# Nikhil-Kulkarni/RayTrace-miniapp

Measured on AMD Instinct MI355X. Metric: ray_steps_per_sec, higher is better.
Workload: dtype f32+f64

## Files before the change

### include/rt_hip.h

```cpp
#ifndef RT_HIP_H
#define RT_HIP_H

#include <stddef.h>
#include <stdint.h>

#ifdef __cplusplus
extern "C" {
#endif

#define RT_N_SUB 3
#define RT_N_FAILED_MAX 32
#define RT_N_SEED_MAX 2

enum {
    RT_OK            = 0,
    RT_ERR_ARG       = 1,
    RT_ERR_NO_DEVICE = 2,
    RT_ERR_HIP       = 3,
    RT_ERR_NOMEM     = 4
};

typedef struct rt_ray {
    float x, y, a, b;
} rt_ray;
// ... 38 lines not shown

int rt_hip_device_count(void);

const char *rt_hip_last_error(void);

int rt_hip_selftest(int device, unsigned long long *n_checked, unsigned long long *n_mismatch);

int rt_hip_image_loop(int device, int N, const rt_beam *beam, const rt_gain *gain,
                      const rt_seed *seed, int method, const rt_ray *rays, size_t n_rays,
                      double scale, double *image, double *I_ang, unsigned int *failure_code,
                      rt_ray *failed_rays, int max_failed, int *n_failed, rt_stats *stats);

int rt_hip_multi_image_loop(int ndev, int N, const rt_beam *beam, const rt_gain *gain, const rt_seed *seed,
                            int method, const rt_ray *rays, size_t n_rays, double scale, double *image,
                            double *I_ang, unsigned int *failure_code, rt_ray *failed_rays, int max_failed,
                            int *n_failed, rt_stats *stats);

int rt_hip_ray_list_grid_dims(const rt_ray *rays, size_t n_rays, int dims[4]);

int rt_hip_multi_last_mode(void);

int rt_hip_host_libm_mode(int device);

void rt_hip_pool_trim(void);

typedef struct rt_hip_plan rt_hip_plan;

int rt_hip_plan_create(rt_hip_plan **plan, int device, int N, const rt_beam *beam,
                       const rt_gain *gain, const rt_seed *seed, int method, double scale);

int rt_hip_plan_set_rays(rt_hip_plan *plan, const rt_ray *rays, size_t n_rays);

int rt_hip_plan_set_ray_grid(rt_hip_plan *plan, const double *gx, int ngx, const double *gy,
                             int ngy, const double *ga, int nga, const double *gb, int ngb,
                             int64_t first, int64_t stride, int64_t count);

int rt_hip_plan_run(rt_hip_plan *plan, void *stream, double *image_dev, double *iang_dev);

int rt_hip_plan_fetch(rt_hip_plan *plan, double *image, double *I_ang,
                      unsigned int *failure_code, rt_ray *failed_rays, int max_failed,
                      int *n_failed, rt_stats *stats);

int rt_hip_plan_kernel_ms(rt_hip_plan *plan, float *ms);

int rt_hip_plan_kernel_times(rt_hip_plan *plan, float *march_ms, float *freq_ms);

int rt_hip_plan_last_fused(rt_hip_plan *plan);

int rt_hip_plan_last_march_instance(rt_hip_plan *plan);

typedef struct rt_hip_run_facts {
    unsigned size;
    int cu_count;
    unsigned long long lds_limit, n_rays, blob_bytes, n_iang;
    unsigned n_tiles;
    int K, Kp, L, rays_per_pixel, n_seed, march_prune, method;
    float c_h3;
    unsigned safe, debug;
    int use_emis, own_cells, exclusive, path_on, spectra_on, step_on, step_one_launch, probe_on, has_ray_list, host_rays,
        tables_bounded, ntest_proven, gv_has_nan;
    int occupancy_per_cu;
    int scan_on;
} rt_hip_run_facts;
typedef struct rt_hip_run_shape {
    unsigned size;
    int kind, lds_tab;
    unsigned n_launch, bthr;
    int mode, bounded, opt, last_march_inst;
    unsigned long long mlds;
    unsigned grid, chunk, park, spin_limit, no_skip, late_first, late_waves, late_chunks;
    int occupancy_asked;
    int maxq, nslot;
    unsigned off_exp, off_iang, off_ctl, off_rem, off_nodes, off_buf, node_cap, n_free, per_wave, split, k_part, n_consumers,
        consumers_first;
    unsigned long long flds, tile_links;
    unsigned fgrid;
    int key_s6, key_emis, key_excl;
    int pass_kind, pass_wg_waves, pass_in_lds, pass_nslot;
    unsigned long long pass_lds;
    unsigned pass_grid, pass_fetch_shift;
} rt_hip_run_shape;
int rt_hip_debug_run_shape(const rt_hip_run_facts *facts, rt_hip_run_shape *out);

int rt_hip_plan_set_timing_ring(rt_hip_plan *plan, int n_runs);
int rt_hip_plan_ring_times(rt_hip_plan *plan, float *march_ms, float *freq_ms, int max_runs, int *n_runs);

double *rt_hip_plan_image_ptr(rt_hip_plan *plan);
double *rt_hip_plan_iang_ptr(rt_hip_plan *plan);

int rt_hip_plan_enable_probe(rt_hip_plan *plan, int on);
int rt_hip_plan_fetch_probe(rt_hip_plan *plan, float *gvl, float *evl, int32_t *ivl,
                            rt_ray *ray2, uint32_t *flags, uint32_t *steps);

int rt_hip_plan_set_exact_emission(rt_hip_plan *plan, int on);

int rt_hip_plan_set_step_factor(rt_hip_plan *plan, double c);

int rt_hip_plan_enable_path(rt_hip_plan *plan, int on);
int rt_hip_plan_fetch_path(rt_hip_plan *plan, float *path, int32_t *err);

int rt_hip_plan_enable_spectra(rt_hip_plan *plan, int on);
int rt_hip_plan_fetch_spectra(rt_hip_plan *plan, double *Iv, rt_ray *ray2, int32_t *err);
double *rt_hip_plan_spectra_ptr(rt_hip_plan *plan);

int rt_hip_plan_enable_length_spectra(rt_hip_plan *plan, int on);
int rt_hip_plan_fetch_length_spectra(rt_hip_plan *plan, int n, double *Iv, rt_ray *ray2, int32_t *err);
int rt_hip_plan_length_spectra_ptrs(rt_hip_plan *plan, int n, double **Iv_dev, rt_ray **ray2_dev, int32_t **err_dev);

int rt_hip_plan_set_spectra_seeds(rt_hip_plan *plan, int n_seed, const rt_seed *seeds);
int rt_hip_plan_fetch_seed_spectra(rt_hip_plan *plan, int s, double *Iv, rt_ray *ray2, int32_t *err);
int rt_hip_plan_seed_spectra_ptrs(rt_hip_plan *plan, int s, double **Iv_dev, rt_ray **ray2_dev, int32_t **err_dev);
int rt_hip_plan_fetch_seed_length_spectra(rt_hip_plan *plan, int s, int n, double *Iv, rt_ray *ray2, int32_t *err);
int rt_hip_plan_seed_length_spectra_ptrs(rt_hip_plan *plan, int s, int n, double **Iv_dev, rt_ray **ray2_dev, int32_t **err_dev);

int rt_hip_plan_set_spectra_ase_seeds(rt_hip_plan *plan, int n_seed, const rt_seed *seeds);
int rt_hip_plan_fetch_full_spectra(rt_hip_plan *plan, int r, double *Iv, rt_ray *ray2, int32_t *err);
int rt_hip_plan_full_spectra_ptrs(rt_hip_plan *plan, int r, double **Iv_dev, rt_ray **ray2_dev, int32_t **err_dev);

int rt_hip_plan_set_length_spectra_ase_seeds(rt_hip_plan *plan, int n_seed, const rt_seed *seeds);
int rt_hip_plan_fetch_full_length_spectra(rt_hip_plan *plan, int r, int n, double *Iv, rt_ray *ray2, int32_t *err);
int rt_hip_plan_full_length_spectra_ptrs(rt_hip_plan *plan, int r, int n, double **Iv_dev, rt_ray **ray2_dev, int32_t **err_dev);

int rt_hip_calc_rays(int device, int N, double dz, const rt_gain *gain, const rt_seed *seed, int K, int method,
                     const double *rays, size_t n, double *Iv, double *ray2, int32_t *err, rt_stats *stats);

int rt_hip_plan_enable_step(rt_hip_plan *plan, int on);
int rt_hip_plan_set_step_buffers(rt_hip_plan *plan, double *E_v_dev, double *nf_dev);
int rt_hip_plan_fetch_step(rt_hip_plan *plan, double *E_v, double *nf, double *I_ang);
int rt_hip_plan_step_ptrs(rt_hip_plan *plan, double **E_v_dev, double **nf_dev);
int rt_hip_multi_step_loop(int ndev, int N, const rt_beam *beam, const rt_gain *gain, const rt_seed *seed, int method,
                           const rt_ray *rays, size_t n_rays, double scale, double *E_v, double *nf, double *I_ang,
                           unsigned int *failure_code, rt_ray *failed_rays, int max_failed, int *n_failed, rt_stats *stats);
int rt_hip_step_loop(int device, int N, const rt_beam *beam, const rt_gain *gain, const rt_seed *seed, int method,
                     const rt_ray *rays, size_t n_rays, double scale, double *E_v, double *nf, double *I_ang,
                     unsigned int *failure_code, rt_ray *failed_rays, int max_failed, int *n_failed, rt_stats *stats);

int rt_hip_plan_set_step_one_launch(rt_hip_plan *plan, int on);

typedef struct rt_gain_values {
    const double *n;
    const float *g0;
    const float *E0;
    const float *gv;
} rt_gain_values;
int rt_hip_plan_update_gain(rt_hip_plan *plan, int N, const rt_gain_values *vals);
int rt_hip_plan_update_gain_dev(rt_hip_plan *plan, int N, const rt_gain_values *vals, void *stream);
int rt_hip_plan_table_flags(rt_hip_plan *plan, int *bounded, int *ntest_proven, int *gv_nonfinite, float *gs_cap);

int rt_hip_plan_set_seeds(rt_hip_plan *plan, int n_seed, const rt_seed *seeds);
int rt_hip_plan_fetch_seed_step(rt_hip_plan *plan, int s, double *E_v, double *nf, double *I_ang,
                                unsigned int *failure_code);
int rt_hip_plan_seed_step_ptrs(rt_hip_plan *plan, int s, double **E_v_dev, double **nf_dev, double **iang_dev);

#define RT_N_SCAN_MAX 32
int rt_hip_plan_enable_length_scan(rt_hip_plan *plan, int on);
int rt_hip_plan_fetch_length_step(rt_hip_plan *plan, int n, double *E_v, double *nf, double *I_ang, unsigned int *failure_code);
int rt_hip_plan_length_step_ptrs(rt_hip_plan *plan, int n, double **E_v_dev, double **nf_dev, double **iang_dev);
int rt_hip_length_scan_loop(int device, int N, const rt_beam *beam, const rt_gain *gain, const rt_seed *seed, int method,
                            const rt_ray *rays, size_t n_rays, double scale, double *E_v, double *nf, double *I_ang,
                            unsigned int *failure_codes, rt_ray *failed_rays, int max_failed, int *n_failed, rt_stats *stats);

int rt_hip_plan_enable_suffix_scan(rt_hip_plan *plan, int on);
int rt_hip_suffix_scan_loop(int device, int N, const rt_beam *beam, const rt_gain *gain, const rt_seed *seed, int method,
                            const rt_ray *rays, size_t n_rays, double scale, double *E_v, double *nf, double *I_ang,
                            unsigned int *failure_codes, rt_ray *failed_rays, int max_failed, int *n_failed, rt_stats *stats);

// ... 71 lines not shown
```

### raytrace-miniapp_amd/backend.py

```python
from __future__ import annotations

import ctypes as C
import subprocess
import time
from pathlib import Path

import numpy as np

from . import cabi
from .problem import Problem, Seed

CSRC = Path(__file__).resolve().parent / "csrc"
LIB_PATH = CSRC / "librt_hip.so"


class RayTraceError(RuntimeError):
    """Raised where the reference calls RAY_ERROR (utilities/RayUtilityMacros.h:88-91)."""


def build_library(force: bool = False) -> Path:
    if force and LIB_PATH.exists():
        LIB_PATH.unlink()
    subprocess.run(["make", "-s", "-C", str(CSRC)], check=True)
    return LIB_PATH
# ... 579 lines not shown
            U, B = C.POINTER(C.c_uint), C.POINTER(C.c_ubyte)
            self.hl.check(self.hl.lib.rt_hip_plan_history_fetch(
                self._h, r, cabi._dp(E_v), cabi._dp(nf), cabi._dp(iang), cabi._dp(es), code.ctypes.data_as(U),
                flags.ctypes.data_as(U), filled.ctypes.data_as(B)), "rt_hip_plan_history_fetch")
            out.append(dict(E_v=E_v, nf=nf, I_ang=iang, E_sum=es, failure_code=code, flags=flags, filled=filled))
        return out

    def fetch_history_sum(self) -> list:
        b, out = self.problem.beam, []
        for r in range(max(1, self.history_info()["n_rec"])):
            E_v, nf, iang, es = np.empty(b.nv), np.empty(b.nx * b.ny), np.empty(b.na * b.nb), np.empty(1)
            self.hl.check(self.hl.lib.rt_hip_plan_history_fetch_sum(self._h, r, cabi._dp(E_v), cabi._dp(nf), cabi._dp(iang),
                                                                    cabi._dp(es)), "rt_hip_plan_history_fetch_sum")
            out.append(dict(E_v=E_v, nf=nf, I_ang=iang, E_sum=float(es[0])))
        return out

    def history_tensors(self) -> list:
        import torch

        b, info, out = self.problem.beam, self.history_info(), []
        T = info["n_steps"]
        for r in range(info["n_rec"]):
            q = [C.c_void_p() for _ in range(6)]
            self.hl.check(self.hl.lib.rt_hip_plan_history_ptrs(self._h, r, *(C.byref(x) for x in q)), "rt_hip_plan_history_ptrs")
            e, n, a, s, c, f = (int(x.value or 0) for x in q)
            words = lambda ptr: _view(ptr, (T // 2 + T % 2,), self.device).view(torch.int32)[:T]
            out.append(dict(E_v=_view(e, (T, b.nv), self.device), nf=_view(n, (T, b.ny, b.nx), self.device),
                            I_ang=_view(a, (T, b.nb, b.na), self.device), E_sum=_view(s, (T,), self.device),
                            failure_code=words(c), flags=words(f)))
        return out

    def history_sum_tensors(self) -> list:
        out = []
        for r in range(self.history_info()["n_rec"]):
            q = [C.c_void_p() for _ in range(4)]
            self.hl.check(self.hl.lib.rt_hip_plan_history_sum_ptrs(self._h, r, *(C.byref(x) for x in q)), "rt_hip_plan_history_sum_ptrs")
            e, n, a, s = (int(x.value or 0) for x in q)
            out.append(dict(**self._record_views((e, n, a)), E_sum=_view(s, (1,), self.device)))
        return out

    def update_gain(self, gain, stream: int | None = None) -> "Plan":
        import copy
        import dataclasses

        old = self.problem.gain
        gv = cabi.GainValues(gain, [(g.Nx, g.Ny) for g in old], self.problem.beam.nv, self.device)
        if gv.on_device:
            if stream is None:
                import torch
                stream = torch.cuda.current_stream(self.device).cuda_stream
            rc = self.hl.lib.rt_hip_plan_update_gain_dev(self._h, gv.N, gv.vals, C.c_void_p(stream))
            self.hl.check(rc, "rt_hip_plan_update_gain_dev")
            self._gain_dev = gv
        else:
            self.hl.check(self.hl.lib.rt_hip_plan_update_gain(self._h, gv.N, gv.vals), "rt_hip_plan_update_gain")
            q = copy.copy(self.problem)
            q.gain = [old[0]] + [dataclasses.replace(old[i], n=t[0], g0=t[1], E0=t[2], gv=t[3]) for i, t in enumerate(gv.tables) if i]
            q.golden_image = q.golden_I_ang = None
            self.problem = q
        return self

    def table_flags(self) -> dict:
        b, t, g, cap = C.c_int(0), C.c_int(0), C.c_int(0), C.c_float(0)
        self.hl.check(self.hl.lib.rt_hip_plan_table_flags(self._h, C.byref(b), C.byref(t), C.byref(g), C.byref(cap)),
                      "rt_hip_plan_table_flags")
        return dict(bounded=b.value, ntest_proven=t.value, gv_nonfinite=g.value, gs_cap=np.float32(cap.value))

    def kernel_ms(self) -> float:
        ms = C.c_float(0)
        self.hl.check(self.hl.lib.rt_hip_plan_kernel_ms(self._h, C.byref(ms)), "rt_hip_plan_kernel_ms")
        return float(ms.value)

    def kernel_times(self) -> tuple:
        a, f = C.c_float(0), C.c_float(0)
        self.hl.check(self.hl.lib.rt_hip_plan_kernel_times(self._h, C.byref(a), C.byref(f)),
                      "rt_hip_plan_kernel_times")
        return float(a.value), float(f.value)

    def last_fused(self) -> bool:
        return bool(self.hl.lib.rt_hip_plan_last_fused(self._h))

    def last_march_instance(self) -> int:
        return int(self.hl.lib.rt_hip_plan_last_march_instance(self._h))

    def set_timing_ring(self, n_runs: int) -> "Plan":
        self.hl.check(self.hl.lib.rt_hip_plan_set_timing_ring(self._h, int(n_runs)), "rt_hip_plan_set_timing_ring")
        self._ring = int(n_runs)
        return self

    def ring_times(self) -> list:
        n = self._ring
        if n < 1:
            return []
        a = np.zeros(n, np.float32)
        f = np.zeros(n, np.float32)
        got = C.c_int(0)
        self.hl.check(self.hl.lib.rt_hip_plan_ring_times(self._h, cabi._fp(a), cabi._fp(f), n, C.byref(got)),
                      "rt_hip_plan_ring_times")
        return [(float(a[i]), float(f[i])) for i in range(got.value)]

    def fetch_probe(self) -> dict:
        n = self.n_rays
        S = (self.problem.N - 1) * cabi.RT_N_SUB
        out = dict(gvl=np.zeros((n, S), np.float32), evl=np.zeros((n, S), np.float32),
                   ivl=np.zeros((n, S), np.int32), ray2=np.zeros(n, cabi.RAY_DTYPE),
                   flags=np.zeros(n, np.uint32), steps=np.zeros(n, np.uint32))
        P = C.POINTER
        rc = self.hl.lib.rt_hip_plan_fetch_probe(
            self._h, cabi._fp(out["gvl"]), cabi._fp(out["evl"]), out["ivl"].ctypes.data_as(P(C.c_int32)),
            cabi.rays_ptr(out["ray2"]), out["flags"].ctypes.data_as(P(C.c_uint32)),
            out["steps"].ctypes.data_as(P(C.c_uint32)))
        self.hl.check(rc, "rt_hip_plan_fetch_probe")
        return out

    @property
    def image_ptr(self) -> int:
        return int(self.hl.lib.rt_hip_plan_image_ptr(self._h) or 0)

    @property
    def iang_ptr(self) -> int:
        return int(self.hl.lib.rt_hip_plan_iang_ptr(self._h) or 0)

    def close(self) -> None:
        if self._h:
            self.hl.lib.rt_hip_plan_destroy(self._h)
            self._h = C.c_void_p()

    def __enter__(self):
        return self

    def __exit__(self, *exc):
        self.close()

    def __del__(self):
        try:
            self.close()
        except Exception:
            pass


def _host_loop(entry: str, problem: Problem, rays, device: int, lead: tuple = (), seeds=None, scales=None, ase: bool = False,
               image: bool = False) -> dict:
    hl = HipLibrary.get()
    m = cabi.Marshalled(problem)
    if rays is None:
        rays = problem.build_rays()
    rays = np.ascontiguousarray(rays, dtype=cabi.RAY_DTYPE)
    b = problem.beam
    sizes = (b.nx * b.ny * b.nv, b.na * b.nb) if image else (b.nv, b.nx * b.ny, b.na * b.nb)
    outs = [np.zeros(lead + (n,)) for n in sizes]
    codes = np.zeros(lead, np.uint32)
    nfail = C.c_int(0)
    failed = np.zeros(cabi.RT_N_FAILED_MAX, dtype=cabi.RAY_DTYPE)
    st = cabi.RtStats()
    args = [device, m.N, C.byref(m.beam), m.gain] + ([] if ase else [m.seed_ref])
    args += [problem.method, cabi.rays_ptr(rays), len(rays), problem.scale]
    if seeds is not None:
        _, arr, _keep = _seed_array(seeds, entry, "a call")
        args += [len(seeds), arr] + ([cabi._dp(scales) if scales is not None else None] if ase else [])
    args += [cabi._dp(o) for o in outs] + [codes.ctypes.data_as(C.POINTER(C.c_uint)), cabi.rays_ptr(failed), cabi.RT_N_FAILED_MAX,
                                          C.byref(nfail), C.byref(st)]
    t0 = time.perf_counter()
    rc = getattr(hl.lib, entry)(*args)
    call_ms = (time.perf_counter() - t0) * 1e3
    hl.check(rc, entry)
    return dict(outs=outs, codes=codes, failure_code=int(np.bitwise_or.reduce(codes, axis=None)), failed_rays=failed[:nfail.value].copy(),
# ... 288 lines not shown
```

### raytrace-miniapp_amd/cabi.py

```python
from __future__ import annotations

import ctypes as C

import numpy as np

RT_N_SUB = 3
RT_N_FAILED_MAX = 32
RT_N_SEED_MAX = 2
RT_N_SCAN_MAX = 32

RT_OK, RT_ERR_ARG, RT_ERR_NO_DEVICE, RT_ERR_HIP, RT_ERR_NOMEM = range(5)

c_double_p = C.POINTER(C.c_double)
c_float_p = C.POINTER(C.c_float)


class RtRay(C.Structure):
    _fields_ = [("x", C.c_float), ("y", C.c_float), ("a", C.c_float), ("b", C.c_float)]


RAY_DTYPE = np.dtype([("x", "<f4"), ("y", "<f4"), ("a", "<f4"), ("b", "<f4")])


class RtBeam(C.Structure):
# ... 252 lines not shown
                                             C.c_int64, C.c_int64, C.c_int64]
    lib.rt_hip_plan_set_ray_grid.restype = C.c_int
    lib.rt_hip_plan_run.argtypes = [vp, vp, vp, vp]
    lib.rt_hip_plan_run.restype = C.c_int
    lib.rt_hip_plan_fetch.argtypes = [vp, c_double_p, c_double_p, P(C.c_uint), P(RtRay), C.c_int,
                                      P(C.c_int), P(RtStats)]
    lib.rt_hip_plan_fetch.restype = C.c_int
    lib.rt_hip_plan_kernel_ms.argtypes = [vp, P(C.c_float)]
    lib.rt_hip_plan_kernel_ms.restype = C.c_int
    lib.rt_hip_plan_kernel_times.argtypes = [vp, P(C.c_float), P(C.c_float)]
    lib.rt_hip_plan_kernel_times.restype = C.c_int
    lib.rt_hip_plan_last_fused.argtypes = [vp]
    lib.rt_hip_plan_last_fused.restype = C.c_int
    if hasattr(lib, "rt_hip_plan_last_march_instance"):
        lib.rt_hip_plan_last_march_instance.argtypes = [vp]
        lib.rt_hip_plan_last_march_instance.restype = C.c_int
    lib.rt_hip_plan_set_timing_ring.argtypes = [vp, C.c_int]
    lib.rt_hip_plan_set_timing_ring.restype = C.c_int
    lib.rt_hip_plan_ring_times.argtypes = [vp, c_float_p, c_float_p, C.c_int, P(C.c_int)]
    lib.rt_hip_plan_ring_times.restype = C.c_int
    lib.rt_hip_plan_image_ptr.argtypes = [vp]
    lib.rt_hip_plan_image_ptr.restype = vp
    lib.rt_hip_plan_iang_ptr.argtypes = [vp]
    lib.rt_hip_plan_iang_ptr.restype = vp
    lib.rt_hip_plan_enable_probe.argtypes = [vp, C.c_int]
    lib.rt_hip_plan_enable_probe.restype = C.c_int
    lib.rt_hip_plan_fetch_probe.argtypes = [vp, c_float_p, c_float_p, P(C.c_int32), P(RtRay),
                                            P(C.c_uint32), P(C.c_uint32)]
    lib.rt_hip_plan_fetch_probe.restype = C.c_int
    lib.rt_hip_plan_set_exact_emission.argtypes = [vp, C.c_int]
    lib.rt_hip_plan_set_exact_emission.restype = C.c_int
    lib.rt_hip_plan_set_step_factor.argtypes = [vp, C.c_double]
    lib.rt_hip_plan_set_step_factor.restype = C.c_int
    lib.rt_hip_plan_enable_path.argtypes = [vp, C.c_int]
    lib.rt_hip_plan_enable_path.restype = C.c_int
    lib.rt_hip_plan_fetch_path.argtypes = [vp, c_float_p, P(C.c_int32)]
    lib.rt_hip_plan_fetch_path.restype = C.c_int
    lib.rt_hip_plan_enable_spectra.argtypes = [vp, C.c_int]
    lib.rt_hip_plan_enable_spectra.restype = C.c_int
    lib.rt_hip_plan_fetch_spectra.argtypes = [vp, c_double_p, P(RtRay), P(C.c_int32)]
    lib.rt_hip_plan_fetch_spectra.restype = C.c_int
    lib.rt_hip_plan_spectra_ptr.argtypes = [vp]
    lib.rt_hip_plan_spectra_ptr.restype = vp
    lib.rt_hip_calc_rays.argtypes = [C.c_int, C.c_int, C.c_double, P(RtGain), P(RtSeed), C.c_int, C.c_int, c_double_p,
                                     C.c_size_t, c_double_p, c_double_p, P(C.c_int32), P(RtStats)]
    lib.rt_hip_calc_rays.restype = C.c_int
    if hasattr(lib, "rt_hip_plan_enable_step"):
        lib.rt_hip_plan_enable_step.argtypes = [vp, C.c_int]
        lib.rt_hip_plan_enable_step.restype = C.c_int
        lib.rt_hip_plan_fetch_step.argtypes = [vp, c_double_p, c_double_p, c_double_p]
        lib.rt_hip_plan_fetch_step.restype = C.c_int
        lib.rt_hip_plan_step_ptrs.argtypes = [vp, P(vp), P(vp)]
        lib.rt_hip_plan_step_ptrs.restype = C.c_int
        lib.rt_hip_step_loop.argtypes = [
            C.c_int, C.c_int, P(RtBeam), P(RtGain), P(RtSeed), C.c_int, P(RtRay), C.c_size_t,
            C.c_double, c_double_p, c_double_p, c_double_p, P(C.c_uint), P(RtRay), C.c_int, P(C.c_int),
            P(RtStats)]
        lib.rt_hip_step_loop.restype = C.c_int
    if hasattr(lib, "rt_hip_multi_step_loop"):
        lib.rt_hip_plan_set_step_buffers.argtypes = [vp, vp, vp]
        lib.rt_hip_plan_set_step_buffers.restype = C.c_int
        lib.rt_hip_multi_step_loop.argtypes = list(lib.rt_hip_step_loop.argtypes)
        lib.rt_hip_multi_step_loop.restype = C.c_int
    if hasattr(lib, "rt_hip_plan_update_gain"):
        lib.rt_hip_plan_update_gain.argtypes = [vp, C.c_int, P(RtGainValues)]
        lib.rt_hip_plan_update_gain.restype = C.c_int
        lib.rt_hip_plan_update_gain_dev.argtypes = [vp, C.c_int, P(RtGainValues), vp]
        lib.rt_hip_plan_update_gain_dev.restype = C.c_int
        lib.rt_hip_plan_table_flags.argtypes = [vp, P(C.c_int), P(C.c_int), P(C.c_int), c_float_p]
        lib.rt_hip_plan_table_flags.restype = C.c_int
    if hasattr(lib, "rt_hip_plan_set_seeds"):
        lib.rt_hip_plan_set_seeds.argtypes = [vp, C.c_int, P(RtSeed)]
        lib.rt_hip_plan_set_seeds.restype = C.c_int
        lib.rt_hip_plan_fetch_seed_step.argtypes = [vp, C.c_int, c_double_p, c_double_p, c_double_p, P(C.c_uint)]
        lib.rt_hip_plan_fetch_seed_step.restype = C.c_int
        lib.rt_hip_plan_seed_step_ptrs.argtypes = [vp, C.c_int, P(vp), P(vp), P(vp)]
        lib.rt_hip_plan_seed_step_ptrs.restype = C.c_int
    if hasattr(lib, "rt_hip_plan_set_step_one_launch"):
        lib.rt_hip_plan_set_step_one_launch.argtypes = [vp, C.c_int]
        lib.rt_hip_plan_set_step_one_launch.restype = C.c_int
    if hasattr(lib, "rt_hip_debug_run_shape"):
        lib.rt_hip_debug_run_shape.argtypes = [P(RtRunFacts), P(RtRunShape)]
        lib.rt_hip_debug_run_shape.restype = C.c_int
    if hasattr(lib, "rt_hip_plan_enable_length_scan"):
        lib.rt_hip_plan_enable_length_scan.argtypes = [vp, C.c_int]
        lib.rt_hip_plan_enable_length_scan.restype = C.c_int
        lib.rt_hip_plan_fetch_length_step.argtypes = [vp, C.c_int, c_double_p, c_double_p, c_double_p, P(C.c_uint)]
        lib.rt_hip_plan_fetch_length_step.restype = C.c_int
        lib.rt_hip_plan_length_step_ptrs.argtypes = [vp, C.c_int, P(vp), P(vp), P(vp)]
        lib.rt_hip_plan_length_step_ptrs.restype = C.c_int
        lib.rt_hip_length_scan_loop.argtypes = list(lib.rt_hip_step_loop.argtypes)
        lib.rt_hip_length_scan_loop.restype = C.c_int
    if hasattr(lib, "rt_hip_plan_enable_suffix_scan"):
        lib.rt_hip_plan_enable_suffix_scan.argtypes = [vp, C.c_int]
        lib.rt_hip_plan_enable_suffix_scan.restype = C.c_int
        lib.rt_hip_suffix_scan_loop.argtypes = list(lib.rt_hip_step_loop.argtypes)
        lib.rt_hip_suffix_scan_loop.restype = C.c_int
    if hasattr(lib, "rt_hip_plan_set_scan_seeds"):
        lib.rt_hip_plan_set_scan_seeds.argtypes = [vp, C.c_int, P(RtSeed)]
        lib.rt_hip_plan_set_scan_seeds.restype = C.c_int
        lib.rt_hip_plan_fetch_seed_length_step.argtypes = [vp, C.c_int, C.c_int, c_double_p, c_double_p, c_double_p, P(C.c_uint)]
        lib.rt_hip_plan_fetch_seed_length_step.restype = C.c_int
        lib.rt_hip_plan_seed_length_step_ptrs.argtypes = [vp, C.c_int, C.c_int, P(vp), P(vp), P(vp)]
        lib.rt_hip_plan_seed_length_step_ptrs.restype = C.c_int
        a = list(lib.rt_hip_step_loop.argtypes)
        lib.rt_hip_seed_length_scan_loop.argtypes = a[:9] + [C.c_int, P(RtSeed)] + a[9:]
        lib.rt_hip_seed_length_scan_loop.restype = C.c_int
    if hasattr(lib, "rt_hip_plan_set_ase_seeds"):
        lib.rt_hip_plan_set_ase_seeds.argtypes = [vp, C.c_int, P(RtSeed), c_double_p]
        lib.rt_hip_plan_set_ase_seeds.restype = C.c_int
        lib.rt_hip_plan_fetch_full_step.argtypes = [vp, C.c_int, c_double_p, c_double_p, c_double_p, P(C.c_uint)]
        lib.rt_hip_plan_fetch_full_step.restype = C.c_int
        lib.rt_hip_plan_full_step_ptrs.argtypes = [vp, C.c_int, P(vp), P(vp), P(vp)]
        lib.rt_hip_plan_full_step_ptrs.restype = C.c_int
        lib.rt_hip_full_step_loop.argtypes = [
            C.c_int, C.c_int, P(RtBeam), P(RtGain), C.c_int, P(RtRay), C.c_size_t, C.c_double, C.c_int, P(RtSeed), c_double_p,
            c_double_p, c_double_p, c_double_p, P(C.c_uint), P(RtRay), C.c_int, P(C.c_int), P(RtStats)]
        lib.rt_hip_full_step_loop.restype = C.c_int
    if hasattr(lib, "rt_hip_plan_set_scan_ase_seeds"):
        lib.rt_hip_plan_set_scan_ase_seeds.argtypes = [vp, C.c_int, P(RtSeed), c_double_p]
        lib.rt_hip_plan_set_scan_ase_seeds.restype = C.c_int
        lib.rt_hip_plan_fetch_full_length_step.argtypes = [vp, C.c_int, C.c_int, c_double_p, c_double_p, c_double_p, P(C.c_uint)]
        lib.rt_hip_plan_fetch_full_length_step.restype = C.c_int
        lib.rt_hip_plan_full_length_step_ptrs.argtypes = [vp, C.c_int, C.c_int, P(vp), P(vp), P(vp)]
        lib.rt_hip_plan_full_length_step_ptrs.restype = C.c_int
        lib.rt_hip_full_length_scan_loop.argtypes = list(lib.rt_hip_full_step_loop.argtypes)
        lib.rt_hip_full_length_scan_loop.restype = C.c_int
    if hasattr(lib, "rt_hip_plan_set_suffix_ase_seeds"):
        lib.rt_hip_plan_set_suffix_ase_seeds.argtypes = [vp, C.c_int, P(RtSeed), c_double_p]
        lib.rt_hip_plan_set_suffix_ase_seeds.restype = C.c_int
        lib.rt_hip_full_suffix_scan_loop.argtypes = list(lib.rt_hip_full_length_scan_loop.argtypes)
        lib.rt_hip_full_suffix_scan_loop.restype = C.c_int
    if hasattr(lib, "rt_hip_plan_set_suffix_seeds"):
        lib.rt_hip_plan_set_suffix_seeds.argtypes = list(lib.rt_hip_plan_set_scan_seeds.argtypes)
        lib.rt_hip_plan_set_suffix_seeds.restype = C.c_int
        lib.rt_hip_seed_suffix_scan_loop.argtypes = list(lib.rt_hip_seed_length_scan_loop.argtypes)
        lib.rt_hip_seed_suffix_scan_loop.restype = C.c_int
    if hasattr(lib, "rt_hip_plan_enable_length_spectra"):
        lib.rt_hip_plan_enable_length_spectra.argtypes = [vp, C.c_int]
        lib.rt_hip_plan_enable_length_spectra.restype = C.c_int
        lib.rt_hip_plan_fetch_length_spectra.argtypes = [vp, C.c_int, c_double_p, P(RtRay), P(C.c_int32)]
        lib.rt_hip_plan_fetch_length_spectra.restype = C.c_int
        lib.rt_hip_plan_length_spectra_ptrs.argtypes = [vp, C.c_int, P(vp), P(vp), P(vp)]
        lib.rt_hip_plan_length_spectra_ptrs.restype = C.c_int
    if hasattr(lib, "rt_hip_plan_set_spectra_seeds"):
        lib.rt_hip_plan_set_spectra_seeds.argtypes = [vp, C.c_int, P(RtSeed)]
        lib.rt_hip_plan_set_spectra_seeds.restype = C.c_int
        lib.rt_hip_plan_fetch_seed_spectra.argtypes = [vp, C.c_int, c_double_p, P(RtRay), P(C.c_int32)]
        lib.rt_hip_plan_fetch_seed_spectra.restype = C.c_int
        lib.rt_hip_plan_seed_spectra_ptrs.argtypes = [vp, C.c_int, P(vp), P(vp), P(vp)]
        lib.rt_hip_plan_seed_spectra_ptrs.restype = C.c_int
        lib.rt_hip_plan_fetch_seed_length_spectra.argtypes = [vp, C.c_int, C.c_int, c_double_p, P(RtRay), P(C.c_int32)]
        lib.rt_hip_plan_fetch_seed_length_spectra.restype = C.c_int
        lib.rt_hip_plan_seed_length_spectra_ptrs.argtypes = [vp, C.c_int, C.c_int, P(vp), P(vp), P(vp)]
        lib.rt_hip_plan_seed_length_spectra_ptrs.restype = C.c_int
    if hasattr(lib, "rt_hip_plan_set_spectra_ase_seeds"):
        lib.rt_hip_plan_set_spectra_ase_seeds.argtypes = [vp, C.c_int, P(RtSeed)]
        lib.rt_hip_plan_set_spectra_ase_seeds.restype = C.c_int
        lib.rt_hip_plan_fetch_full_spectra.argtypes = [vp, C.c_int, c_double_p, P(RtRay), P(C.c_int32)]
        lib.rt_hip_plan_fetch_full_spectra.restype = C.c_int
        lib.rt_hip_plan_full_spectra_ptrs.argtypes = [vp, C.c_int, P(vp), P(vp), P(vp)]
        lib.rt_hip_plan_full_spectra_ptrs.restype = C.c_int
    if hasattr(lib, "rt_hip_plan_set_length_spectra_ase_seeds"):
        lib.rt_hip_plan_set_length_spectra_ase_seeds.argtypes = [vp, C.c_int, P(RtSeed)]
        lib.rt_hip_plan_set_length_spectra_ase_seeds.restype = C.c_int
        lib.rt_hip_plan_fetch_full_length_spectra.argtypes = [vp, C.c_int, C.c_int, c_double_p, P(RtRay), P(C.c_int32)]
        lib.rt_hip_plan_fetch_full_length_spectra.restype = C.c_int
        lib.rt_hip_plan_full_length_spectra_ptrs.argtypes = [vp, C.c_int, C.c_int, P(vp), P(vp), P(vp)]
        lib.rt_hip_plan_full_length_spectra_ptrs.restype = C.c_int
    if hasattr(lib, "rt_hip_plan_history_create"):
        up, bp = P(C.c_uint), P(C.c_ubyte)
        lib.rt_hip_plan_history_create.argtypes = [vp, C.c_int]
        lib.rt_hip_plan_history_create.restype = C.c_int
        lib.rt_hip_plan_history_append.argtypes = [vp, C.c_int, C.c_double, C.c_int, vp]
        lib.rt_hip_plan_history_append.restype = C.c_int
        lib.rt_hip_plan_history_ptrs.argtypes = [vp, C.c_int, P(vp), P(vp), P(vp), P(vp), P(vp), P(vp)]
        lib.rt_hip_plan_history_ptrs.restype = C.c_int
        lib.rt_hip_plan_history_sum_ptrs.argtypes = [vp, C.c_int, P(vp), P(vp), P(vp), P(vp)]
        lib.rt_hip_plan_history_sum_ptrs.restype = C.c_int
        lib.rt_hip_plan_history_fetch.argtypes = [vp, C.c_int, c_double_p, c_double_p, c_double_p, c_double_p, up, up, bp]
        lib.rt_hip_plan_history_fetch.restype = C.c_int
        lib.rt_hip_plan_history_fetch_sum.argtypes = [vp, C.c_int, c_double_p, c_double_p, c_double_p, c_double_p]
        lib.rt_hip_plan_history_fetch_sum.restype = C.c_int
        lib.rt_hip_plan_history_info.argtypes = [vp, P(C.c_int), P(C.c_int), P(C.c_int)]
        lib.rt_hip_plan_history_info.restype = C.c_int
        lib.rt_hip_debug_history_layout.argtypes = [P(RtHistoryFacts), P(RtHistoryLayout)]
        lib.rt_hip_debug_history_layout.restype = C.c_int
    lib.rt_hip_plan_set_debug.argtypes = [vp, C.c_uint]
    lib.rt_hip_plan_set_debug.restype = C.c_int
    lib.rt_hip_plan_destroy.argtypes = [vp]
    lib.rt_hip_plan_destroy.restype = None


HIP_API_SYMBOLS = [
    "rt_hip_device_count", "rt_hip_last_error", "rt_hip_selftest", "rt_hip_image_loop", "rt_hip_multi_image_loop",
    "rt_hip_multi_last_mode", "rt_hip_ray_list_grid_dims", "rt_hip_host_libm_mode", "rt_hip_pool_trim", "rt_hip_plan_create",
    "rt_hip_plan_set_rays", "rt_hip_plan_set_ray_grid", "rt_hip_plan_run", "rt_hip_plan_fetch",
    "rt_hip_plan_kernel_ms", "rt_hip_plan_kernel_times", "rt_hip_plan_last_fused", "rt_hip_plan_last_march_instance", "rt_hip_plan_set_timing_ring", "rt_hip_plan_ring_times", "rt_hip_plan_image_ptr", "rt_hip_plan_iang_ptr", "rt_hip_plan_enable_probe",
    "rt_hip_plan_fetch_probe", "rt_hip_plan_set_exact_emission", "rt_hip_plan_set_step_factor", "rt_hip_plan_enable_path",
    "rt_hip_plan_fetch_path", "rt_hip_plan_enable_spectra", "rt_hip_plan_fetch_spectra", "rt_hip_plan_spectra_ptr",
    "rt_hip_calc_rays", "rt_hip_plan_enable_step", "rt_hip_plan_fetch_step", "rt_hip_plan_step_ptrs", "rt_hip_step_loop",
    "rt_hip_plan_set_step_buffers", "rt_hip_multi_step_loop",
    "rt_hip_plan_update_gain", "rt_hip_plan_update_gain_dev", "rt_hip_plan_table_flags",
    "rt_hip_plan_set_seeds", "rt_hip_plan_fetch_seed_step", "rt_hip_plan_seed_step_ptrs",
    "rt_hip_plan_enable_length_scan", "rt_hip_plan_fetch_length_step", "rt_hip_plan_length_step_ptrs", "rt_hip_length_scan_loop",
    "rt_hip_plan_set_scan_seeds", "rt_hip_plan_fetch_seed_length_step", "rt_hip_plan_seed_length_step_ptrs",
    "rt_hip_seed_length_scan_loop",
    "rt_hip_plan_enable_suffix_scan", "rt_hip_suffix_scan_loop",
    "rt_hip_plan_set_ase_seeds", "rt_hip_plan_fetch_full_step", "rt_hip_plan_full_step_ptrs", "rt_hip_full_step_loop",
    "rt_hip_plan_set_scan_ase_seeds", "rt_hip_plan_fetch_full_length_step", "rt_hip_plan_full_length_step_ptrs",
    "rt_hip_full_length_scan_loop",
    "rt_hip_plan_set_suffix_ase_seeds", "rt_hip_full_suffix_scan_loop",
    "rt_hip_plan_set_suffix_seeds", "rt_hip_seed_suffix_scan_loop",
    "rt_hip_plan_enable_length_spectra", "rt_hip_plan_fetch_length_spectra", "rt_hip_plan_length_spectra_ptrs",
    "rt_hip_plan_set_spectra_seeds", "rt_hip_plan_fetch_seed_spectra", "rt_hip_plan_seed_spectra_ptrs",
    "rt_hip_plan_fetch_seed_length_spectra", "rt_hip_plan_seed_length_spectra_ptrs",
    "rt_hip_plan_set_spectra_ase_seeds", "rt_hip_plan_fetch_full_spectra", "rt_hip_plan_full_spectra_ptrs",
    "rt_hip_plan_set_length_spectra_ase_seeds", "rt_hip_plan_fetch_full_length_spectra", "rt_hip_plan_full_length_spectra_ptrs",
    "rt_hip_plan_set_step_one_launch", "rt_hip_debug_run_shape",
    "rt_hip_plan_history_create", "rt_hip_plan_history_append", "rt_hip_plan_history_ptrs", "rt_hip_plan_history_sum_ptrs",
    "rt_hip_plan_history_fetch", "rt_hip_plan_history_fetch_sum", "rt_hip_plan_history_info", "rt_hip_debug_history_layout",
    "rt_hip_plan_set_debug", "rt_hip_plan_destroy",
]
```

### raytrace-miniapp_amd/csrc/rt_blob_pack.h

```cpp
#pragma once

#include <cmath>
#include <cstring>
#include <vector>

#include "rt_device.h"

namespace rt {

inline BlobGain blob_pack_length(std::vector<unsigned char> &blob, size_t i, int Nx, int Ny, const double *x, const double *y,
                                 const double *n, const float *g0, const float *E0, bool &tiny_spacing, bool &bad_index)
{
    const size_t npix = (size_t) Nx * (size_t) Ny;
    BlobGain h;
    memset(&h, 0, sizeof(h));
    h.lo_x     = (float) x[0];
    h.hi_x     = (float) x[Nx - 1];
    h.lo_y     = (float) y[0];
    h.hi_y     = (float) y[Ny - 1];
    h.mirror_y = 0;
    if (h.lo_y >= 0) {
        h.lo_y     = -h.hi_y;
        h.mirror_y = 1;
    }
    h.Nx  = Nx;
    h.Ny  = Ny;
    h.x0f = (float) x[0];
    h.y0f = (float) y[0];
    const double ihx = (double) (Nx - 1) / (x[Nx - 1] - x[0]);
    const double ihy = (double) (Ny - 1) / (y[Ny - 1] - y[0]);
    h.inv_hxf        = std::isfinite(ihx) && fabs(ihx) < 1e30 ? (float) ihx : 0.0f;
    h.inv_hyf        = std::isfinite(ihy) && fabs(ihy) < 1e30 ? (float) ihy : 0.0f;
    auto put_intervals = [&](const double *gp, int n, bool mirrored) {
        const int off = (int) blob.size();
        blob.resize(blob.size() + sizeof(Interval) * (size_t) n);
        Interval *iv = reinterpret_cast<Interval *>(blob.data() + off);
        memset(iv, 0, sizeof(Interval) * (size_t) n);
        for (int k = 1; k < n; k++) {
            const double lo = gp[k - 1], hi = gp[k], hk = hi - lo;
            if (!(hk >= 1e-30))
                tiny_spacing = true;
            iv[k].lo   = lo;
            iv[k].hi   = hi;
            iv[k].rh   = 1.0 / hk;
            iv[k].rw   = 1.0 / (double) (float) hk;
            iv[k].w    = (float) hk;
            iv[k].b_lo = (float) (lo - 0.1 * hk);
            iv[k].b_hi = (float) (hi + 0.1 * hk);
            if (mirrored && k == 1)
                iv[k].b_lo = -iv[k].b_hi;
        }
        return off;
    };
    h.off_ix   = put_intervals(x, Nx, false);
    h.off_iy   = put_intervals(y, Ny, h.mirror_y != 0);
    h.off_node = (int) blob.size();
    blob.resize(blob.size() + sizeof(Node) * npix);
    Node *nd = reinterpret_cast<Node *>(blob.data() + h.off_node);
    for (size_t c = 0; c < npix; c++) {
        if (!std::isfinite((float) n[c]))
            bad_index = true;
        nd[c].n  = n[c];
        nd[c].g0 = g0[c];
        nd[c].E0 = E0 ? E0[c] : 0.0f;
    }
    memcpy(blob.data() + sizeof(BlobGain) * i, &h, sizeof(h));
    return h;
}

}
```

### raytrace-miniapp_amd/csrc/rt_device.h

```cpp
#pragma once

#include <hip/hip_runtime.h>
#include <stdint.h>

#include "../../include/rt_hip.h"

namespace rt {

constexpr int WAVE = 64;

struct alignas(16) Node {
    double n;
    float g0;
    float E0;
};

struct DevGain {
    const float *gv;
};

struct alignas(16) BlobGain {
    float lo_x, hi_x, lo_y, hi_y;
    int Nx, Ny, mirror_y, off_ix;
    int off_iy, off_node, pad0, pad1;
    float x0f, y0f;
    float inv_hxf, inv_hyf;
};

struct alignas(16) Interval {
    double lo;
    double rw;
    float w;
    float b_lo;
    float b_hi;
    float pad;
    double hi;
    double rh;
};

struct DevSeed {
    const double *x[5];
    const double *f[5];
    int dim[5];
    int pad;
    double f0;
};

struct DevBeam {
    const double *x, *y, *a, *b, *dv;
    int nx, ny, na, nb, nv;
    int pad;
    double dx, dy, da, db;
    double inv_dx, inv_dy, inv_da, inv_db;
    double g_first[4], g_last[4];
};

struct DevRays {
    const rt_ray *list;
    const float *sxy;
    const double *gx, *gy, *ga, *gb;
    const float *tan_a, *tan_b;
    const double *sf;
    const unsigned char *sin;
    int ngx, ngy, nga, ngb;
    long long first, stride;
    unsigned long long count;
    unsigned div_mul[3], div_sh[3];
};

struct RecSlot {
    float g, e;
    int c;
};
struct RecMeta {
    float px, py, sx, sy, sz;
    unsigned flags_steps;
};

struct DevCtl {
    unsigned int next_tile[8][8][16];
    unsigned int next_tile_f[4][8][16];
    unsigned int failure_code;
    unsigned int n_failed;
    unsigned long long cell_steps;
    unsigned long long n_escaped;
    unsigned long long n_skipped;
    unsigned long long n_rays;
    rt_ray failed[RT_N_FAILED_MAX];
    unsigned int seed_code[RT_N_SEED_MAX];
    unsigned int len_code[RT_N_SCAN_MAX];
    unsigned int seed_len_code[RT_N_SEED_MAX][RT_N_SCAN_MAX];
    unsigned int rec_code[RT_N_SEED_MAX + 2];
    unsigned int rec_len_code[1 + RT_N_SEED_MAX][RT_N_SCAN_MAX];
};

struct DevProbe {
    rt_ray *ray2;
    uint32_t *flags;
    uint32_t *steps;
};

struct DevParams {
    int N, L, K, method;
    int use_emis, has_seed;
    float dz0;
    int probe_on;
    int Kp;
    int exact_emis;
    double scale;
    DevBeam beam;
    DevSeed seed;
    const DevGain *gain;
    DevRays rays;
    double *image;
    double *iang;
    DevCtl *ctl;
    DevProbe probe;
    unsigned int n_tiles;
    unsigned int tile_begin, tile_end, freq_id;
    unsigned int ray_begin, ray_end, launch_id, pad_launch;
    unsigned int debug;
// ... 103 lines not shown
```

### raytrace-miniapp_amd/csrc/rt_launch.hip

```cpp
#include "rt_path.hip"
#include "rt_freq.hip"
#include "rt_fused.hip"
#include "rt_spec.hip"
#include "rt_step.hip"
#include "rt_step_seeds.hip"
#include "rt_fused_step.hip"
#include "rt_step_scan.hip"
#include "rt_step_rscan.hip"
#include "rt_step_scan_seeds.hip"
#include "rt_step_ase_seeds.hip"
#include "rt_step_scan_ase_seeds.hip"
#include "rt_step_rscan_ase_seeds.hip"

#include "rt_step_rscan_seeds.hip"
#include "rt_spec_scan.hip"
#include "rt_spec_seeds.hip"
#include "rt_spec_scan_seeds.hip"
#include "rt_spec_ase_seeds.hip"
#include "rt_spec_scan_ase_seeds.hip"

#include "rt_runtime.h"
#include "rt_run_shape.h"

#include <atomic>
// ... 103 lines not shown
void (*step_kernel(bool s6, bool emis))(const rt::StepKArg)
{
    return emis ? (s6 ? rt::rt_step_kernel<6, true> : rt::rt_step_kernel<0, true>) : (s6 ? rt::rt_step_kernel<6, false> : rt::rt_step_kernel<0, false>);
}
void (*seeds_kernel(bool s6))(const rt::SeedsKArg) { return s6 ? rt::rt_step_seeds_kernel<6> : rt::rt_step_seeds_kernel<0>; }
void (*ase_seeds_kernel(bool s6))(const rt::AseSeedsKArg) { return s6 ? rt::rt_step_ase_seeds_kernel<6> : rt::rt_step_ase_seeds_kernel<0>; }
void (*scan_kernel(bool emis))(const rt::ScanKArg) { return emis ? rt::rt_step_scan_kernel<true> : rt::rt_step_scan_kernel<false>; }
void (*rscan_kernel(bool emis))(const rt::ScanKArg) { return emis ? rt::rt_step_rscan_kernel<true> : rt::rt_step_rscan_kernel<false>; }
void (*spec_scan_kernel(bool emis, bool backward))(const rt::SpecScanKArg)
{
    return emis ? (backward ? rt::rt_spec_scan_kernel<true, true> : rt::rt_spec_scan_kernel<true, false>)
                : (backward ? rt::rt_spec_scan_kernel<false, true> : rt::rt_spec_scan_kernel<false, false>);
}
void (*spec_seeds_kernel(bool s6))(const rt::SpecSeedsKArg) { return s6 ? rt::rt_spec_seeds_kernel<6> : rt::rt_spec_seeds_kernel<0>; }
void (*spec_ase_seeds_kernel(bool s6))(const rt::SpecSeedsKArg) { return s6 ? rt::rt_spec_ase_seeds_kernel<6> : rt::rt_spec_ase_seeds_kernel<0>; }
void (*spec_scan_seeds_kernel(bool backward))(const rt::SpecScanSeedsKArg)
{
    return backward ? rt::rt_spec_scan_seeds_kernel<true> : rt::rt_spec_scan_seeds_kernel<false>;
}
void (*spec_scan_ase_seeds_kernel(bool backward))(const rt::SpecScanSeedsKArg)
{
    return backward ? rt::rt_spec_scan_ase_seeds_kernel<true> : rt::rt_spec_scan_ase_seeds_kernel<false>;
}

struct PassRun {
    unsigned tile_begin, tile_end, freq_id;
    unsigned safe;
    unsigned char *bad;
};

rt::FreqKArg freq_args(const rt_hip_plan *p, bool iang_in_lds, int nslot, unsigned fetch_shift, const PassRun &r)
{
    const rt::DevParams &P = p->P;
    rt::FreqKArg a;
    memset(&a, 0, sizeof(a));
    a.hot.gv0        = p->gv_dev.size() > 1 ? p->gv_dev[1] : nullptr;
    a.hot.gv1        = p->gv_dev.size() > 2 ? p->gv_dev[2] : nullptr;
    a.hot.gain       = P.gain;
    a.hot.rec        = P.rec;
    a.hot.image      = P.image;
    a.hot.iang       = P.iang;
    a.hot.ctl        = P.ctl;
    a.hot.dv2        = p->dv2_dev;
    a.hot.seed_fk    = P.has_seed ? P.seed.f[4] : p->dv2_dev;
    a.hot.bad        = r.bad;
    a.hot.scale      = P.scale;
    a.hot.gs_cap     = P.gs_cap;
    a.hot.K          = P.K;
    a.hot.Kp         = P.Kp;
    a.hot.L          = P.L;
    a.hot.method     = P.method;
    a.hot.rec_stride = P.rec_stride;
    a.hot.n_rays     = (unsigned) P.rays.count;
    a.hot.tile_begin = r.tile_begin;
    a.hot.tile_end   = r.tile_end;
    a.hot.freq_id    = r.freq_id;
    a.hot.fetch_shift = fetch_shift;
    a.hot.nslot      = nslot;
    a.hot.nx         = P.beam.nx;
    a.hot.ny         = P.beam.ny;
    a.hot.n_ang      = P.beam.na * P.beam.nb;
    a.hot.flags      = (P.exclusive ? rt::FQ_EXCLUSIVE : 0u) | (r.safe == 1 ? rt::FQ_SAFE_CHECK : 0u) |
                  (r.safe == 2 ? rt::FQ_SAFE_SKIP : 0u) | (P.exact_emis ? rt::FQ_EXACT_EMIS : 0u) |
                  (P.has_seed ? rt::FQ_HAS_SEED : 0u) | (P.probe_on ? rt::FQ_PROBE : 0u) |
                  (p->gv_has_nan ? rt::FQ_GV_NAN : 0u) | (iang_in_lds ? rt::FQ_IANG_LDS : 0u) |
                  ((P.method != 1 || P.has_seed || P.probe_on) ? rt::FQ_NEED_EXIT : 0u) |
                  (P.own_cells ? rt::FQ_OWN_CELLS : 0u) | ((P.debug & 4u) ? rt::FQ_DBG_NOFLUSH : 0u);
    a.cold.beam  = P.beam;
    a.cold.seed  = P.seed;
    a.cold.rays  = P.rays;
    a.cold.probe = P.probe;
    return a;
}

RunFacts run_facts(const rt_hip_plan *p)
{
    const rt::DevParams &P = p->P;
    RunFacts f;
    f.cu_count        = p->cu_count;
    f.lds_limit       = p->lds_limit;
    f.n_rays          = p->n_rays;
    f.n_tiles         = P.n_tiles;
    f.blob_bytes      = P.blob_bytes;
    f.K               = P.K;
    f.Kp              = P.Kp;
    f.L               = P.L;
    f.n_iang          = p->n_iang;
    f.rays_per_pixel  = P.rays.nga * P.rays.ngb;
    f.n_seed          = p->scan_on ? p->n_scan_seed : p->n_seed;
    if (p->n_spec_seed > 0)
        f.n_seed = p->n_spec_seed;
    f.c_h3            = P.c_h3;
    f.march_prune     = p->march_prune;
    f.method          = P.method;
    f.safe            = P.safe;
    f.debug           = P.debug;
    f.use_emis        = P.use_emis != 0;
    f.own_cells       = P.own_cells != 0;
    f.exclusive       = P.exclusive != 0;
    f.path_on         = p->path_on;
    f.spectra_on      = p->spectra_on;
    f.step_on         = p->step_on;
    f.step_one_launch = p->step_one_launch;
    f.probe_on        = p->probe_on;
    f.has_ray_list    = P.rays.list != nullptr;
    f.host_rays       = p->host_rays != nullptr;
    f.tables_bounded  = p->tables_bounded;
    f.ntest_proven    = p->ntest_proven;
    f.gv_has_nan      = p->gv_has_nan;
    f.scan_on         = p->scan_on && p->step_on;
    f.length_spectra_on = p->lspec_on;
    return f;
}

template <typename KArg> KArg pass_args(const rt::FreqKArg &fa)
{
    KArg a;
    memset(&a, 0, sizeof(a));
    a.hot       = fa.hot;
    a.hot.image = nullptr;
    a.cold      = fa.cold;
    return a;
}

rt::SeedRec seed_rec(const rt_hip_plan *p, int r)
{
    double *blk = p->recs_dev + (size_t) r * p->recs_stride;
    return rt::SeedRec{ blk, blk + p->recs_nf_off, blk + p->recs_ang_off };
}
void fill_scan(rt::ScanArg &a, const rt_hip_plan *p) { a = rt::ScanArg{ p->scan_bnd, p->recs_dev, p->recs_stride, p->recs_nf_off, p->recs_ang_off }; }
int fill_seed_tabs(rt::SeedTabs &tb, const rt_hip_plan *p, int n_seed, bool grid_tabs, const char *who)
{
    for (int i = 0; i < n_seed; i++) {
        tb.fk[i]   = p->seed_set[i].f[4];
        tb.sf[i]   = grid_tabs ? p->seedset_sf[i] : nullptr;
        tb.sin[i]  = grid_tabs ? p->seedset_sin[i] : nullptr;
        tb.seed[i] = p->seed_set[i];
        if (grid_tabs && (!tb.sf[i] || !tb.sin[i]))
            return fail_arg((std::string(who) + " were not built for this ray grid").c_str());
    }
    return RT_OK;
}

bool seeds_on_grid(const rt_hip_plan *p, const RecordKindRow &k)
{
    return k.ase ? p->P.rays.gx && !p->P.rays.list && p->P.method != 1 && p->seedset_sf[0] != nullptr : p->P.rays.sf != nullptr;
}
int records_ready(const rt_hip_plan *p, const RunFacts &f, const RecordSet &R)
{
    const RecordKindRow &k = R.row();
    auto fail = [&](const char *what) { return fail_arg((std::string("step kernel of ") + k.name + what).c_str()); };
    if (!p->recs_dev || (k.lengths && !p->scan_bnd))
        return fail(": the records or the boundary states of this run were not allocated");
    if (p->recs_doubles < (size_t) R.n_rec() * p->recs_stride)
        return fail(": the records of this run are smaller than the blocks of its kind");
    if (k.lengths && f.L > RT_N_SCAN_MAX)
        return fail(": more than RT_N_SCAN_MAX lengths");
    if (k.seeds && (f.n_seed < 1 || f.n_seed > RT_N_SEED_MAX || f.use_emis != k.ase || (k.suffix && f.method != 1)))
        return fail(": not 1 .. RT_N_SEED_MAX seeds on the plan (emission or gain-only, forward or backward) the kind takes");
    return RT_OK;
}
template <typename KArg> KArg records_args(const rt::FreqKArg &fa, const RecordKindRow &k)
{
    KArg a = pass_args<KArg>(fa);
    if (k.lengths)
        a.hot.iang = nullptr;
// ... 292 lines not shown
        if (p->path_rays != (size_t) p->n_rays || !p->path_dev) {
            (void) hipFree(p->path_dev);
            (void) hipFree(p->path_err);
            p->path_dev = nullptr;
            p->path_err = nullptr;
            HIP_TRY(dev_malloc((void **) &p->path_dev, (size_t) p->n_rays * n2 * 3 * sizeof(float) + 16));
            HIP_TRY(hipMalloc((void **) &p->path_err, (size_t) p->n_rays * sizeof(int32_t) + 16));
            p->path_rays = (size_t) p->n_rays;
        }
        HIP_TRY(hipMemsetAsync(p->path_dev, 0, (size_t) p->n_rays * n2 * 3 * sizeof(float), stream));
        HIP_TRY(hipMemsetAsync(p->path_err, 0, (size_t) p->n_rays * sizeof(int32_t), stream));
        p->P.path     = p->path_dev;
        p->P.path_err = p->path_err;
    }
    const RowSet R = row_set(run_facts(p));
    const size_t n = (size_t) p->n_rays, rows = n * (size_t) R.n_blocks();
    if (R.any() && !R.lengths()) {
        rt::SpecOut &o = p->spec[p->spec_sel];
        if (p->spec_rays[p->spec_sel] < rows || !o.Iv) {
            plan_quiesce(p);
            (void) hipFree(o.Iv);
            o = {};
            p->spec_rays[p->spec_sel] = 0;
            const size_t iv_bytes = align_up(rows * (size_t) p->P.K * sizeof(double) + 16, 256), r2_bytes = align_up(rows * sizeof(rt_ray) + 16, 256);
            unsigned char *b = nullptr;
            HIP_TRY(dev_malloc((void **) &b, iv_bytes + r2_bytes + rows * sizeof(int32_t) + 16));
            o.Iv   = reinterpret_cast<double *>(b);
            o.ray2 = reinterpret_cast<rt_ray *>(b + iv_bytes);
            o.err  = reinterpret_cast<int32_t *>(b + iv_bytes + r2_bytes);
            p->spec_rays[p->spec_sel] = rows;
        }
    }
    if (R.lengths()) {
        const size_t iv_bytes = align_up(rows * (size_t) p->P.K * sizeof(double) + 16, 256), r2_bytes = align_up((size_t) R.n_ray2_blocks() * n * sizeof(rt_ray) + 16, 256);
        const size_t need_ls  = iv_bytes + r2_bytes + rows * sizeof(int32_t) + 16;
        if (need_ls > p->lspec_bytes || !p->lspec_dev) {
            plan_quiesce(p);
            pool_free(p->device, p->lspec_dev);
            p->lspec_dev   = nullptr;
            p->lspec_bytes = 0;
            p->lspec       = {};
            const hipError_t e = pool_alloc(p->device, (void **) &p->lspec_dev, need_ls);
            if (e == hipErrorOutOfMemory) {
                (void) hipGetLastError();
                fail_arg("length spectra: the rows of every length (L n K 8 bytes) do not fit into device memory");
                return RT_ERR_NOMEM;
            }
            HIP_TRY(e);
            p->lspec_bytes = need_ls;
        }
        p->lspec.Iv   = reinterpret_cast<double *>(p->lspec_dev);
        p->lspec.ray2 = reinterpret_cast<rt_ray *>(p->lspec_dev + iv_bytes);
        p->lspec.err  = reinterpret_cast<int32_t *>(p->lspec_dev + iv_bytes + r2_bytes);
    }
    if (s.kind != RUN_TWO_KERNELS && (p->tile_next_n < s.tile_links || !p->tile_next)) {
        plan_quiesce(p);
        pool_free(p->device, p->tile_next);
        p->tile_next = nullptr;
        HIP_TRY(pool_alloc(p->device, (void **) &p->tile_next, s.tile_links * sizeof(unsigned) + 16));
        p->tile_next_n = s.tile_links;
    }
    return RT_OK;
}

static rt::DevParams run_params(const rt_hip_plan *p, const RunShape &s)
{
    rt::DevParams P = p->P;
    P.chunk       = s.chunk;
    P.park        = s.park;
    P.path_on     = p->path_on ? 1u : 0u;
    P.spin_limit  = s.spin_limit;
    P.no_skip     = s.no_skip;
    P.late_first  = s.late_first;
    P.late_waves  = s.late_waves;
    P.late_chunks = s.late_chunks;
    P.ray_begin   = 0;
    P.ray_end     = (unsigned) p->n_rays;
    P.launch_id   = 0;
    if (s.opt & rt::MARCH_OPT_SCAN) {
        const unsigned long long b = (unsigned long long) (uintptr_t) p->scan_bnd;
        P.pad_march[0]             = (unsigned) (b & 0xffffffffull);
        P.pad_march[1]             = (unsigned) (b >> 32);
    }
    return P;
}

static int launch_one(rt_hip_plan *p, const RunFacts &f, const RunShape &s, const rt::DevParams &P, hipStream_t stream)
{
    const rt::FreqKArg fa = freq_args(p, true, s.nslot, s.fetch_shift, PassRun{ 0, f.n_tiles, 0, 0, nullptr });
    if (s.kind == RUN_STEP_ONE_LAUNCH) {
        rt::FusedStepKArg sa;
        memset(&sa, 0, sizeof(sa));
        sa.P           = P;
        sa.S           = pass_args<rt::StepKArg>(fa);
        sa.S.out       = p->step;
        sa.tile_next   = p->tile_next;
        sa.lay         = s.lay;
        return launch(p, fused_step_kernel(s.bounded, f.s6(), s.opt), s.fgrid, s.bthr, s.flds, stream, sa);
    }
    rt::FusedKArg a;
    a.P         = P;
    a.F         = fa;
    a.tile_next = p->tile_next;
    a.lay       = s.lay;
    return launch(p, fused_kernel(s.bounded, f.s6(), s.maxq, s.emis, s.opt), s.fgrid, s.bthr, s.flds, stream, a);
}

static int launch_march(rt_hip_plan *p, const RunShape &s, rt::DevParams &P, hipStream_t stream)
{
    const march_fn kernel = march_kernel(s.lds_tab, s.bounded, s.mode, s.opt);
    for (unsigned c = 0; c < s.n_launch && s.grid > 0 && !(P.debug & 2u); c++) {
        const unsigned long long b = p->n_rays * c / s.n_launch, e = p->n_rays * (c + 1) / s.n_launch;
        if (p->host_rays) {
            HIP_TRY(hipMemcpy(p->rays_dev + b, p->host_rays + b, (size_t) (e - b) * sizeof(rt_ray), hipMemcpyHostToDevice));
            if (tan_mode(p->device) == 2) {
                std::vector<float> h((size_t) (e - b) * 2);
                host_tangents(p->host_rays + b, (size_t) (e - b), h.data());
                HIP_TRY(hipMemcpy(p->tan_dev + 2 * b, h.data(), h.size() * sizeof(float), hipMemcpyHostToDevice));
            } else {
                hipLaunchKernelGGL(rt::rt_tan_kernel, dim3((unsigned) ((e - b + 255) / 256)), dim3(256), 0, stream,
                                   p->rays_dev + b, (unsigned long long) (e - b), p->tan_dev + 2 * b);
                HIP_TRY(hipGetLastError());
            }
        }
        if (s.n_launch > 1)
            P.chunk = march_chunk(e - b, s.grid, s.bthr);
        P.ray_begin = (unsigned) b;
        P.ray_end   = (unsigned) e;
        P.launch_id = c;
        const int rc = launch(p, kernel, s.grid, s.bthr, s.mlds, stream, P);
        if (rc != RT_OK)
            return rc;
    }
    return RT_OK;
}

static int launch_second(rt_hip_plan *p, const RunFacts &f, const Tuning &t, const rt::DevParams &P, hipStream_t stream)
{
    const PassKind kind = pass_kind(f);
    if (kind == PASS_PATH) {
        if (p->n_rays) {
            hipLaunchKernelGGL(rt::rt_path_kernel, dim3((unsigned) ((p->n_rays + 255) / 256)), dim3(256), 0, stream, P);
            HIP_TRY(hipGetLastError());
        }
        return RT_OK;
    }
    if (!spectra_pass(kind) && (f.debug & 1u))
        return RT_OK;
    return launch_pass(p, f, t, kind, stream);
}

int plan_launch_run(rt_hip_plan *p, hipStream_t stream)
{
    if (p->n_rays > (unsigned long long) MAX_LIST_RAYS)
        return fail_arg("more than 2^32 - 4096 rays in one run");
    const RunFacts f = run_facts(p);
    const Tuning t   = read_tuning();
    int rc           = RT_OK;
    const RunShape s = run_shape(f, t, [&](const RunShape &m) { return march_occupancy(p, m, rc); });
    if (rc != RT_OK)
        return rc;
    p->last_march_inst = s.last_march_inst;
    if ((rc = ensure_buffers(p, s, stream)) != RT_OK)
        return rc;
    HIP_TRY(hipEventRecord(p->ev0, stream));
    p->last_fused  = false;
    rt::DevParams P = run_params(p, s);
    const bool one = s.kind != RUN_TWO_KERNELS;
    if ((rc = one ? launch_one(p, f, s, P, stream) : launch_march(p, s, P, stream)) != RT_OK)
        return rc;
    p->host_rays = nullptr;
    HIP_TRY(hipEventRecord(p->evm, stream));
    if (!one && (rc = launch_second(p, f, t, P, stream)) != RT_OK)
        return rc;
    HIP_TRY(hipEventRecord(p->ev1, stream));
    p->last_fused = one;
    return RT_OK;
}

}

extern "C" {

int rt_hip_debug_run_shape(const rt_hip_run_facts *facts, rt_hip_run_shape *out)
{
    if (!facts || !out || facts->size != sizeof(rt_hip_run_facts) || out->size != sizeof(rt_hip_run_shape))
        return fail_arg("rt_hip_debug_run_shape: NULL argument or a size field that is not this library's sizeof");
    if (facts->cu_count < 1 || facts->lds_limit == 0)
        return fail_arg("rt_hip_debug_run_shape: cu_count < 1 or lds_limit == 0");
    RunFacts f;
    f.cu_count        = facts->cu_count;
    f.lds_limit       = (size_t) facts->lds_limit;
    f.n_rays          = facts->n_rays;
    f.n_tiles         = facts->n_tiles;
    f.blob_bytes      = (size_t) facts->blob_bytes;
    f.K               = facts->K;
    f.Kp              = facts->Kp;
    f.L               = facts->L;
    f.n_iang          = (size_t) facts->n_iang;
    f.rays_per_pixel  = facts->rays_per_pixel;
    f.n_seed          = facts->n_seed;
    f.c_h3            = facts->c_h3;
    f.march_prune     = facts->march_prune;
    f.method          = facts->method;
    f.safe            = facts->safe;
    f.debug           = facts->debug;
    f.use_emis        = facts->use_emis != 0;
    f.own_cells       = facts->own_cells != 0;
    f.exclusive       = facts->exclusive != 0;
    f.path_on         = facts->path_on != 0;
    f.spectra_on      = facts->spectra_on != 0;
    f.step_on         = facts->step_on != 0;
    f.step_one_launch = facts->step_one_launch != 0;
    f.probe_on        = facts->probe_on != 0;
    f.has_ray_list    = facts->has_ray_list != 0;
    f.host_rays       = facts->host_rays != 0;
    f.tables_bounded  = facts->tables_bounded != 0;
    f.ntest_proven    = facts->ntest_proven != 0;
    f.gv_has_nan      = facts->gv_has_nan != 0;
    f.scan_on         = facts->scan_on != 0;
    f.length_spectra_on = facts->spectra_on == 2;
    f.spectra_on        = facts->spectra_on != 0 && facts->spectra_on != 2;
    const Tuning t    = read_tuning();
    const RunShape s  = run_shape(f, t, [&](const RunShape &) { return facts->occupancy_per_cu; });
    const unsigned size = out->size;
    memset(out, 0, sizeof(*out));
    out->size            = size;
    out->kind            = (int) s.kind;
    out->lds_tab         = s.lds_tab;
    out->n_launch        = s.n_launch;
    out->bthr            = s.bthr;
    out->mode            = s.mode;
    out->bounded         = s.bounded;
    out->opt             = s.opt;
    out->last_march_inst = s.last_march_inst;
    out->mlds            = s.mlds;
    out->grid            = s.grid;
    out->chunk           = s.chunk;
    out->park            = s.park;
    out->spin_limit      = s.spin_limit;
    out->no_skip         = s.no_skip;
    out->late_first      = s.late_first;
    out->late_waves      = s.late_waves;
    out->late_chunks     = s.late_chunks;
    out->occupancy_asked = s.occupancy_asked;
    out->key_s6          = f.s6();
    out->key_emis        = f.use_emis;
    out->key_excl        = f.use_emis && f.exclusive;
    if (s.kind != RUN_TWO_KERNELS) {
        out->maxq            = s.maxq;
        out->nslot           = s.nslot;
        out->off_exp         = s.lay.off_exp;
        out->off_iang        = s.lay.off_iang;
        out->off_ctl         = s.lay.off_ctl;
        out->off_rem         = s.lay.off_rem;
        out->off_nodes       = s.lay.off_nodes;
        out->off_buf         = s.lay.off_buf;
        out->node_cap        = s.lay.node_cap;
        out->n_free          = s.lay.n_free;
        out->per_wave        = s.lay.per_wave;
        out->split           = s.lay.split;
        out->k_part          = s.lay.k_part;
        out->n_consumers     = s.lay.n_consumers;
        out->consumers_first = s.lay.consumers_first;
        out->flds            = s.flds;
        out->tile_links      = s.tile_links;
        out->fgrid           = s.fgrid;
        out->pass_kind       = s.kind == RUN_STEP_ONE_LAUNCH ? (int) PASS_STEP : (int) PASS_FREQ;
        out->pass_wg_waves   = (int) (s.bthr / 64);
        out->pass_in_lds     = 1;
        out->pass_nslot      = s.nslot;
        out->pass_lds        = s.flds;
        out->pass_grid       = s.fgrid;
        out->pass_fetch_shift = s.fetch_shift;
        return RT_OK;
    }
    const PassKind kind   = pass_kind(f);
    const PassShape ps    = pass_shape(kind, f, t);
    out->pass_kind        = (int) kind;
    out->pass_wg_waves    = ps.wg_waves;
    out->pass_in_lds      = ps.in_lds;
    out->pass_nslot       = ps.nslot;
    out->pass_lds         = ps.lds;
    out->pass_grid        = ps.grid;
    out->pass_fetch_shift = ps.fetch_shift;
    return RT_OK;
}

#ifdef RT_WAVETIMES
int rt_hip_debug_wavetimes(unsigned long long *summary8, unsigned long long *end8192, unsigned long long *dry8192)
{
    HIP_TRY(hipDeviceSynchronize());
    HIP_TRY(hipMemcpyFromSymbol(summary8, HIP_SYMBOL(rt::g_wt), 8 * sizeof(unsigned long long)));
    HIP_TRY(hipMemcpyFromSymbol(end8192, HIP_SYMBOL(rt::g_wt_end), 8192 * sizeof(unsigned long long)));
    HIP_TRY(hipMemcpyFromSymbol(dry8192, HIP_SYMBOL(rt::g_wt_dry), 8192 * sizeof(unsigned long long)));
    unsigned long long init[8] = { ~0ull, 0, ~0ull, 0, ~0ull, 0, 0, 0 };
    HIP_TRY(hipMemcpyToSymbol(HIP_SYMBOL(rt::g_wt), init, sizeof(init)));
    return RT_OK;
}
int rt_hip_debug_wavetrace(unsigned long long *trace, int samples, unsigned *blocks)
{
    HIP_TRY(hipDeviceSynchronize());
    if (samples != rt::WT_TRACE)
        return fail_arg("rt_hip_debug_wavetrace: samples");
    if (blocks)
        HIP_TRY(hipMemcpyFromSymbol(blocks, HIP_SYMBOL(rt::g_wt_blocks), sizeof(unsigned) * 8192 * rt::WT_TRACE * 6));
    HIP_TRY(hipMemcpyFromSymbol(trace, HIP_SYMBOL(rt::g_wt_trace), sizeof(unsigned long long) * 8192 * rt::WT_TRACE));
    void *sym = nullptr;
    HIP_TRY(hipGetSymbolAddress(&sym, HIP_SYMBOL(rt::g_wt_trace)));
    HIP_TRY(hipMemset(sym, 0, sizeof(unsigned long long) * 8192 * rt::WT_TRACE));
    return RT_OK;
}
int rt_hip_debug_publish(unsigned long long *pub4, unsigned long long *vm)
{
    HIP_TRY(hipDeviceSynchronize());
    HIP_TRY(hipMemcpyFromSymbol(pub4, HIP_SYMBOL(rt::g_wt_pub), sizeof(unsigned long long) * 8192 * 4));
    HIP_TRY(hipMemcpyFromSymbol(vm, HIP_SYMBOL(rt::g_wt_vm), sizeof(unsigned long long) * 8192));
    void *sym = nullptr;
    HIP_TRY(hipGetSymbolAddress(&sym, HIP_SYMBOL(rt::g_wt_pub)));
    HIP_TRY(hipMemset(sym, 0, sizeof(unsigned long long) * 8192 * 4));
    HIP_TRY(hipGetSymbolAddress(&sym, HIP_SYMBOL(rt::g_wt_vm)));
    HIP_TRY(hipMemset(sym, 0, sizeof(unsigned long long) * 8192));
    return RT_OK;
}
int rt_hip_debug_freqtimes(unsigned long long *times, unsigned *n_waves)
{
    HIP_TRY(hipDeviceSynchronize());
    HIP_TRY(hipMemcpyFromSymbol(times, HIP_SYMBOL(rt::g_ft), 6 * 8192 * sizeof(unsigned long long)));
    HIP_TRY(hipMemcpyFromSymbol(n_waves, HIP_SYMBOL(rt::g_ft_n), sizeof(unsigned)));
    const unsigned zero = 0;
    HIP_TRY(hipMemcpyToSymbol(HIP_SYMBOL(rt::g_ft_n), &zero, sizeof(zero)));
    return RT_OK;
}
#endif

#ifdef RT_INSTRUMENT
int rt_hip_debug_ray_iters(unsigned short *out, unsigned long long n)
{
    HIP_TRY(hipDeviceSynchronize());
    HIP_TRY(hipMemcpyFromSymbol(out, HIP_SYMBOL(rt::g_ray_iters), (size_t) n * sizeof(unsigned short)));
    return RT_OK;
}
#endif
#ifdef RT_INSTRUMENT
int rt_hip_debug_prune_counters(unsigned long long *out4)
{
    HIP_TRY(hipDeviceSynchronize());
    HIP_TRY(hipMemcpyFromSymbol(out4, HIP_SYMBOL(rt::g_prune), 4 * sizeof(unsigned long long)));
    unsigned long long z[4] = { 0 };
    HIP_TRY(hipMemcpyToSymbol(HIP_SYMBOL(rt::g_prune), z, sizeof(z)));
    return RT_OK;
}
#endif
#ifdef RT_TIMEBLOCKS
int rt_hip_debug_retire_counters(unsigned long long *out4)
{
    HIP_TRY(hipDeviceSynchronize());
    HIP_TRY(hipMemcpyFromSymbol(out4, HIP_SYMBOL(rt::g_retire), 4 * sizeof(unsigned long long)));
    unsigned long long z[4] = { 0 };
    HIP_TRY(hipMemcpyToSymbol(HIP_SYMBOL(rt::g_retire), z, sizeof(z)));
    return RT_OK;
}
#endif
#if defined(RT_INSTRUMENT) || defined(RT_TIMEBLOCKS)
int rt_hip_debug_counters(unsigned long long *out8)
{
    HIP_TRY(hipDeviceSynchronize());
    HIP_TRY(hipMemcpyFromSymbol(out8, HIP_SYMBOL(rt::g_inst), 8 * sizeof(unsigned long long)));
    unsigned long long z[8] = { 0 };
    HIP_TRY(hipMemcpyToSymbol(HIP_SYMBOL(rt::g_inst), z, sizeof(z)));
    return RT_OK;
// ... 5 lines not shown
```

### raytrace-miniapp_amd/csrc/rt_march.hip

```cpp
#pragma once
#include "rt_math.h"

#include <cfloat>

namespace rt {

enum : int { ST_DONE = -1, ST_IDLE = 0, ST_CELL = 1, ST_XSETUP = 2, ST_STEP = 3 };

typedef double f64x2 __attribute__((ext_vector_type(2)));
typedef float f32x4 __attribute__((ext_vector_type(4)));
typedef unsigned u32x4 __attribute__((ext_vector_type(4)));

__device__ __forceinline__ unsigned div_magic(unsigned x, unsigned mul, unsigned sh)
{
    return mul ? __umulhi(x, mul) >> sh : x;
}
__device__ __forceinline__ void grid_index(const DevRays &R, unsigned ridx, unsigned &i, unsigned &j, unsigned &k,
                                           unsigned &m)
{
    const unsigned ijkm = (unsigned) (R.first + (long long) ridx * R.stride);
    const unsigned q1   = div_magic(ijkm, R.div_mul[0], R.div_sh[0]);
    m                   = ijkm - q1 * (unsigned) R.ngb;
    const unsigned q2   = div_magic(q1, R.div_mul[1], R.div_sh[1]);
    k                   = q1 - q2 * (unsigned) R.nga;
    i                   = div_magic(q2, R.div_mul[2], R.div_sh[2]);
    j                   = q2 - i * (unsigned) R.ngy;
}

__device__ __forceinline__ void load_ray(const DevRays &R, unsigned ridx, rt_ray &ray, float &ta, float &tb,
                                         bool want_tan)
{
    if (R.list) {
        ray = R.list[ridx];
        if (want_tan) {
            ta = R.sxy[2 * (size_t) ridx];
            tb = R.sxy[2 * (size_t) ridx + 1];
        }
    } else {
        unsigned i, j, k, m;
        grid_index(R, ridx, i, j, k, m);
        ray.x      = (float) R.gx[i];
        ray.y      = (float) R.gy[j];
        ray.a      = (float) R.ga[k];
        ray.b      = (float) R.gb[m];
        if (want_tan) {
            ta = R.tan_a[k];
            tb = R.tan_b[m];
        }
    }
}

__device__ __attribute__((noinline)) float tan_wide(float x)
{
    if (!(fabsf(x) <= FLT_MAX))
        return x - x;
    return (float) tan((double) x);
}
__device__ __attribute__((noinline)) float atan_wide(float x)
{
    const float A0 = 3.3333334327e-01f, A1 = -2.0000000298e-01f, A2 = 1.4285714924e-01f, A3 = -1.1111110449e-01f,
                A4 = 9.0908870101e-02f, A5 = -7.6918758452e-02f, A6 = 6.6610731184e-02f, A7 = -5.8335702866e-02f,
                A8 = 4.9768779427e-02f, A9 = -3.6531571299e-02f, A10 = 1.6285819933e-02f;
    const unsigned hx = __float_as_uint(x), ix = hx & 0x7fffffffu;
    const bool neg = (hx >> 31) != 0u;
    if (ix >= 0x4c000000u) {
        if (ix > 0x7f800000u)
            return x + x;
        const float r = 1.5707962513e+00f + 7.5497894159e-08f;
        return neg ? -r : r;
    }
    float hi, lo;
    x = fabsf(x);
    if (ix < 0x3f980000u) {
        if (ix < 0x3f300000u) {
            hi = 4.6364760399e-01f;
            lo = 5.0121582440e-09f;
            x  = (2.0f * x - 1.0f) / (2.0f + x);
        } else {
            hi = 7.8539812565e-01f;
            lo = 3.7748947079e-08f;
            x  = (x - 1.0f) / (x + 1.0f);
        }
    } else {
        if (ix < 0x401c0000u) {
            hi = 9.8279368877e-01f;
            lo = 3.4473217170e-08f;
            x  = (x - 1.5f) / (1.0f + 1.5f * x);
        } else {
            hi = 1.5707962513e+00f;
            lo = 7.5497894159e-08f;
            x  = -1.0f / x;
        }
    }
    const float z = x * x, w = z * z;
    const float s1 = z * (A0 + w * (A2 + w * (A4 + w * (A6 + w * (A8 + w * A10)))));
    const float s2 = w * (A1 + w * (A3 + w * (A5 + w * (A7 + w * A9))));
    const float r  = hi - ((x * (s1 + s2) - lo) - x);
    return neg ? -r : r;
}

__device__ __attribute__((noinline)) float ktanf_flt32(float x, float y, int iy)
{
    const float T[13] = { 3.3333334327e-01f, 1.3333334029e-01f, 5.3968254477e-02f, 2.1869488060e-02f, 8.8632395491e-03f,
                          3.5920790397e-03f, 1.4562094584e-03f, 5.8804126456e-04f, 2.4646313977e-04f, 7.8179444245e-05f,
                          7.1407252108e-05f, -1.8558637748e-05f, 2.5907305826e-05f };
    const float pio4 = 7.8539812565e-01f, pio4lo = 3.7748947079e-08f;
    float z, r, v, w, s;
    const int hx = (int) __float_as_uint(x), ix = hx & 0x7fffffff;
    if (ix < 0x39000000) {
        if ((int) x == 0) {
            if ((ix | (iy + 1)) == 0)
                return 1.0f / fabsf(x);
            else if (iy == 1)
                return x;
            else
                return -1.0f / x;
        }
    }
    if (ix >= 0x3f2ca140) {
        if (hx < 0) {
            x = -x;
            y = -y;
        }
        z = pio4 - x;
        w = pio4lo - y;
        x = z + w;
        y = 0.0f;
        if (fabsf(x) < 0x1p-13f)
            return (1 - ((hx >> 30) & 2)) * iy * (1.0f - 2 * iy * x);
    }
    z = x * x;
// ... 619 lines not shown
#ifndef RT_ABL_NOMETA
                *reinterpret_cast<RecMeta *>(metap) = m;
#else
                if (m.px == 1234.5f)
                    *reinterpret_cast<RecMeta *>(metap) = m;
#endif
                diag.ray_retired(ridx);
                tot_steps += steps;
                tot_esc += escaped ? 1u : 0u;
                tot_skip += (fl & F_SKIP) ? 1u : 0u;
                tot_rays++;
                st = ST_IDLE;
                if (FUSED) {
                    if (__hip_atomic_fetch_add(&done.rem[cslot], 0xffffffffu, __ATOMIC_RELAXED, __HIP_MEMORY_SCOPE_WAVEFRONT) == 1u) {
                        diag.publish_begin();
                        asm volatile("s_waitcnt vmcnt(0)" ::: "memory");
                        diag.publish_stores_landed();
                        tile_publish(done, ridx >> 6);
                        diag.publish_end();
                    }
                }
            }
            diag.mark(3);
            if (more) {
                diag.refill();
                const int rank = (int) __builtin_amdgcn_mbcnt_hi((unsigned) (idle >> 32),
                                                                 __builtin_amdgcn_mbcnt_lo((unsigned) idle, 0u));
                int need = n_idle, off = 0;
                bool got = false;
                while (need > 0) {
                    if (chunk_next == chunk_end && !(FUSED && chunk_next != fetched_end)) {
                        unsigned c = 0;
                        if (lane == 0)
                            c = atomicAdd(&P.ctl->next_tile[P.launch_id][shard][zone * 8u], 1u);
                        c = (unsigned) __builtin_amdgcn_readfirstlane((int) c) * 8u + shard + zone * n_main;
                        if (c >= (zone ? n_chunks : n_main)) {
                            if (++shards_seen_empty == 8) {
                                if (zone == 0u && late_wave && n_main < n_chunks) {
                                    zone              = 1u;
                                    shards_seen_empty = 0;
                                    continue;
                                }
                                more = false;
                                refill_at = 0u;
                                diag.counters_dry();
                                break;
                            }
                            shard = (shard + 1) & 7u;
                            continue;
                        }
                        chunk_next = P.ray_begin + c * CH;
                        chunk_end  = (n_rays - chunk_next < CH) ? n_rays : chunk_next + CH;
                        if (FUSED) {
                            fetched_end = chunk_end;
                            chunk_end   = chunk_next;
                        }
                    }
                    if (FUSED && chunk_next == chunk_end) {
                        const unsigned in_use    = lane < 32 ? __hip_atomic_load(&done.rem[lane], __ATOMIC_RELAXED, __HIP_MEMORY_SCOPE_WAVEFRONT) : 1u;
                        const unsigned slot_busy = ~(unsigned) __ballot(lane < 32 && in_use == 0u);
                        const int fs = __builtin_ffs((int) ~slot_busy) - 1;
                        if (fs < 0)
                            break;
                        chunk_end = fetched_end - chunk_next < (unsigned) WAVE ? fetched_end : chunk_next + (unsigned) WAVE;
                        cur_slot  = (unsigned) fs;
                        if (lane == 0)
                            __hip_atomic_store(&done.rem[fs], chunk_end - chunk_next, __ATOMIC_RELAXED, __HIP_MEMORY_SCOPE_WAVEFRONT);
                    }
                    int avail = (int) (chunk_end - chunk_next);
                    int take  = avail < need ? avail : need;
                    if (st == ST_IDLE && !got && rank >= off && rank < off + take) {
                        ridx = chunk_next + (unsigned) (rank - off);
                        got  = true;
                        if (FUSED)
                            cslot = cur_slot;
                    }
                    chunk_next += (unsigned) take;
                    need -= take;
                    off += take;
                }
                if (!BOUNDED && __ballot(got) != 0ull)
                    spin = 0;
                if (got) {
                    rt_ray ray;
                    float ta = 0, tb = 0;
                    load_ray(P.rays, ridx, ray, ta, tb, true);
                    px = ray.x;
                    py = ray.y;
                    pz = 0.0f;
                    sx = ta;
                    sy = tb;
                    sz = 1.0f;
                    if (backward) {
                        sx = -sx;
                        sy = -sy;
                        sz = -sz;
                    }
                    renormalise(sx, sy, sz);
                    const BlobGain G0 = hdr[backward ? P.N - 1 : 1];
                    const float dsum  = sx + sy + sz;
                    const bool wild   = ((px != px) | (py != py) | (dsum != dsum)) &
                                      !((px < G0.lo_x) | (px > G0.hi_x) | (py < G0.lo_y) | (py > G0.hi_y));
                    if (path_on) {
                        float *pp = P.path + (size_t) ridx * 3 * (size_t) (S + 1) + 3 * (size_t) (backward ? S : 0);
                        pp[0]     = px;
                        pp[1]     = py;
                    }
                    recp      = P.rec + rec_slot_off(ridx, backward ? S - 1 : 0, P.rec_stride);
                    lane12    = (ridx & 63u) * 12u;
                    seg       = 0;
                    iz        = 0;
                    ii        = backward ? P.N - 1 : 1;
                    G         = G0;
                    z         = 0.0f;
                    z_stop    = zs0;
                    gacc      = 0.0f;
                    eacc      = 0.0f;
                    cell_last = 0;
                    steps     = 0;
                    escaped   = wild;
                    sx        = wild ? 0.0f : sx;
                    sy        = wild ? 0.0f : sy;
                    sz        = wild ? 0.0f : sz;
                    any_bits  = P.no_skip;
                    sub       = 0;
                    st        = ST_CELL;
                }
                idle2 = __ballot(st == ST_IDLE);
            }
        }
        if (idle2 == ~0ull) {
            if (!more)
                break;
        } else {

        diag.mark(0);
        const unsigned long long want_a = __ballot(st == ST_CELL);
        int park_at = (int) P.park;
        if (!more || (int) P.park > 12 || REFILL > 8) {
            const int n_live = WAVE - (int) __popcll(idle2);
            const int fifth  = (n_live * 13 + 63) >> 6;
            park_at          = fifth < (int) P.park ? fifth : (int) P.park;
        }
        const bool do_a = (int) __popcll(want_a) >= park_at || (~(idle2 | want_a)) == 0ull;
        diag.blocks_run(do_a && want_a != 0ull, st == ST_XSETUP);
        if (do_a && st == ST_CELL) {
            bool in_seg        = !escaped & (z < 0.995f * z_stop);
            if (!in_seg) {
#ifndef RT_ABL_NOSTORE
                *reinterpret_cast<RecSlot *>(recp) = RecSlot{ gacc, eacc, cell_last };
#endif
                recp += backward ? -(int) REC_SLOT_ROW : (int) REC_SLOT_ROW;
                any_bits |= (__float_as_uint(gacc) | __float_as_uint(eacc)) & 0x7fffffffu;
                if (path_on) {
                    float *pp = P.path + (size_t) ridx * 3 * (size_t) (S + 1);
                    for (int zz = iz; zz < (escaped ? RT_N_SUB : iz + 1); zz++) {
                        const int idx = RT_N_SUB * (ii - 1) + (backward ? RT_N_SUB - zz - 1 : zz + 1);
                        pp[3 * idx]     = px;
                        pp[3 * idx + 1] = py;
                    }
                }
                gacc      = 0.0f;
                eacc      = 0.0f;
                cell_last = 0;
                sub++;
                const bool wrap = iz == RT_N_SUB - 1;
                const bool fin  = escaped | (sub == S);
                iz              = wrap ? 0 : iz + 1;
                z               = wrap ? 0.0f : z;
                st              = fin ? ST_DONE : ST_CELL;
                diag.finishing(st);
// ... 88 lines not shown
```

### raytrace-miniapp_amd/csrc/rt_plan.hip

```cpp
#include "rt_runtime.h"
#include "rt_blob_pack.h"

#include <algorithm>
#include <cfloat>
#include <cmath>
#include <cstdio>
#include <cstdlib>
#include <cstring>
#include <memory>
#include <mutex>
#include <string>
#include <thread>

using namespace rtr;

namespace {

struct ArenaBuilder {
    unsigned char *base = nullptr;
    size_t cap = 0, used = 0;
    bool pinned = false, overflow = false;
    std::unique_ptr<unsigned char[]> own;
    ArenaBuilder() = default;
    ArenaBuilder(const ArenaBuilder &) = delete;
// ... 179 lines not shown
                       const rt_seed *seed, int method, double scale)
{
    return rtr::plan_create_on(out, nullptr, device, N, beam, gain, seed, method, scale);
}

}

int rtr::plan_create_on(rt_hip_plan **out, hipStream_t upload_q, int device, int N, const rt_beam *beam, const rt_gain *gain,
                        const rt_seed *seed, int method, double scale)
{
    if (!out || !beam || !gain)
        return fail_arg("rt_hip_plan_create: NULL argument");
    *out = nullptr;
    if (N < 2)
        return fail_arg("rt_hip_plan_create: need at least 2 lengths");
    if (method != 1 && method != 2)
        return fail_arg("rt_hip_plan_create: method must be 1 (backward) or 2 (forward)");
    if (beam->nx < 1 || beam->ny < 1 || beam->na < 1 || beam->nb < 1 || beam->nv < 1)
        return fail_arg("rt_hip_plan_create: empty beam grid");
    const int L = N - 1;
    if (L > 64)
        return fail_arg("rt_hip_plan_create: more than 65 lengths are not supported");
    const int K = beam->nv;
    for (int i = 1; i < N; i++) {
        if (gain[i].Nx < 2 || gain[i].Ny < 2 || !gain[i].x || !gain[i].y || !gain[i].n || !gain[i].g0 ||
            !gain[i].gv)
            return fail_arg("rt_hip_plan_create: incomplete gain table");
        if (gain[i].Nv != K)
            return fail_arg("rt_hip_plan_create: gain.Nv != beam.nv");
    }
    int ndev = rt_hip_device_count();
    if (ndev <= 0) {
        last_error() = "no HIP device";
        return RT_ERR_NO_DEVICE;
    }
    if (device < 0 || device >= ndev)
        return fail_arg("rt_hip_plan_create: bad device index");
    HIP_TRY(hipSetDevice(device));

    rt_hip_plan *p = new rt_hip_plan();
    p->t_created   = std::chrono::steady_clock::now();
    p->device      = device;
    {
        static std::mutex mu;
        static std::vector<std::pair<int, int>> known;
        std::lock_guard<std::mutex> lock(mu);
        if ((size_t) device >= known.size())
            known.resize((size_t) device + 1, { 0, 0 });
        if (known[(size_t) device].first == 0) {
            int n = 0, lds = 0;
            hipError_t e = hipDeviceGetAttribute(&n, hipDeviceAttributeMultiprocessorCount, device);
            if (e == hipSuccess)
                e = hipDeviceGetAttribute(&lds, hipDeviceAttributeMaxSharedMemoryPerBlock, device);
            if (e != hipSuccess || n < 1 || lds < 1) {
                delete p;
                return fail_hip(e, "hipDeviceGetAttribute(multiprocessor count, LDS per work-group)", __FILE__, __LINE__);
            }
            known[(size_t) device] = { n, lds };
        }
        p->cu_count  = known[(size_t) device].first;
        p->lds_limit = (size_t) known[(size_t) device].second;
    }

    static const bool timing = getenv("RT_HIP_TIMING") != nullptr;
    auto t_prev = std::chrono::steady_clock::now();
    auto lap    = [&](const char *what) {
        if (timing) {
            const auto now = std::chrono::steady_clock::now();
            fprintf(stderr, "    plan_create %-18s %7.3f ms\n", what, std::chrono::duration<double, std::milli>(now - t_prev).count());
            t_prev = now;
        }
    };
    lap("device");
    ArenaBuilder ab;
    {
        auto piece      = [](size_t bytes) { return align_up(bytes, 256) + 256; };
        const size_t kp = (size_t) ((K + 3) & ~3);
        size_t capacity = piece(sizeof(rt::DevGain) * (size_t) N), blob_bytes = align_up(sizeof(rt::BlobGain) * (size_t) N, 16);
        for (int i = 1; i < N; i++) {
            const size_t cells = (size_t) gain[i].Nx * (size_t) gain[i].Ny;
            capacity += piece(cells * kp * sizeof(float));
            blob_bytes += sizeof(rt::Interval) * ((size_t) gain[i].Nx + (size_t) gain[i].Ny) + sizeof(rt::Node) * cells;
        }
        capacity += piece(blob_bytes);
        capacity += piece(sizeof(double) * (size_t) beam->nx) + piece(sizeof(double) * (size_t) beam->ny) +
                    piece(sizeof(double) * (size_t) beam->na) + piece(sizeof(double) * (size_t) beam->nb) + 2 * piece(sizeof(double) * kp);
        if (seed)
            for (int i = 0; i < 5; i++)
                capacity += 2 * piece(sizeof(double) * ((size_t) (seed->dim[i] > 0 ? seed->dim[i] : 0) + kp));
        ab.start(capacity, upload_q != nullptr);
    }
    std::vector<rt::DevGain> dg((size_t) N);
    std::vector<size_t> off_gv((size_t) N, 0);
    const bool use_emis = gain[0].E0 != nullptr && seed == nullptr;
    const int Kp = (K + 3) & ~3;
    for (int i = 1; i < N; i++) {
        const size_t cells = (size_t) gain[i].Nx * (size_t) gain[i].Ny;
        if (cells * (size_t) Kp * sizeof(float) >= (1ull << 32)) {
            delete p;
            return fail_arg("rt_hip_plan_create: a lineshape table of 4 GiB or more is not supported");
        }
        if (Kp == K) {
            off_gv[(size_t) i] = ab.put(gain[i].gv, sizeof(float) * cells * (size_t) K);
        } else {
            off_gv[(size_t) i] = ab.reserve(sizeof(float) * cells * (size_t) Kp);
            float *dst         = reinterpret_cast<float *>(ab.base + off_gv[(size_t) i]);
            for (size_t c = 0; c < cells; c++)
                memcpy(dst + c * (size_t) Kp, gain[i].gv + c * (size_t) K, sizeof(float) * (size_t) K);
        }
    }
    const size_t off_bx  = ab.put(beam->x, sizeof(double) * (size_t) beam->nx);
    const size_t off_by  = ab.put(beam->y, sizeof(double) * (size_t) beam->ny);
    const size_t off_ba  = ab.put(beam->a, sizeof(double) * (size_t) beam->na);
    const size_t off_bb  = ab.put(beam->b, sizeof(double) * (size_t) beam->nb);
    const size_t off_bdv = ab.reserve(sizeof(double) * (size_t) Kp);
    memcpy(ab.base + off_bdv, beam->dv, sizeof(double) * (size_t) beam->nv);
    const size_t off_bdv2 = ab.reserve(sizeof(double) * (size_t) Kp);
    for (int k = 0; k < beam->nv; k++) {
        const double d2 = 2.0 * beam->dv[k];
        memcpy(ab.base + off_bdv2 + sizeof(double) * (size_t) k, &d2, sizeof(double));
    }
    size_t off_sx[5] = { 0 }, off_sf[5] = { 0 };
    if (seed) {
        for (int i = 0; i < 5; i++) {
            if (seed->dim[i] < (i < 4 ? 2 : 1) || !seed->x[i] || !seed->f[i]) {
                delete p;
                return fail_arg("rt_hip_plan_create: incomplete seed table");
            }
            if (i == 4 && seed->dim[4] != K) {
                delete p;
                return fail_arg("rt_hip_plan_create: seed.dim[4] != beam.nv");
            }
            off_sx[i] = ab.put(seed->x[i], sizeof(double) * (size_t) seed->dim[i]);
            if (i == 4) {
                off_sf[i] = ab.reserve(sizeof(double) * (size_t) Kp);
                memcpy(ab.base + off_sf[i], seed->f[i], sizeof(double) * (size_t) seed->dim[i]);
            } else {
                off_sf[i] = ab.put(seed->f[i], sizeof(double) * (size_t) seed->dim[i]);
            }
        }
    }
    const size_t off_gain = ab.reserve(sizeof(rt::DevGain) * (size_t) N);
    std::vector<unsigned char> blob(align_up(sizeof(rt::BlobGain) * (size_t) N, 16));
    bool tiny_spacing = false, bad_index = false, all_bounded = true, ntest_proven = true;
    p->tab.assign((size_t) N, rt_hip_plan::TableShape());
    for (int i = 1; i < N; i++) {
        const rt_gain &g  = gain[i];
        const rt::BlobGain h = rt::blob_pack_length(blob, (size_t) i, g.Nx, g.Ny, g.x, g.y, g.n, g.g0, g.E0, tiny_spacing, bad_index);
        {
            double n_lo = g.n[0], n_hi = g.n[0], dn = 0.0, w_min = g.x[1] - g.x[0];
            for (int k = 1; k < g.Nx; k++)
                w_min = std::min(w_min, g.x[k] - g.x[k - 1]);
            for (int k = 1; k < g.Ny; k++)
                w_min = std::min(w_min, g.y[k] - g.y[k - 1]);
            for (int iy = 0; iy < g.Ny; iy++) {
                const double *row = g.n + (size_t) iy * (size_t) g.Nx;
                for (int ix = 0; ix < g.Nx; ix++) {
                    n_lo = std::min(n_lo, row[ix]);
                    n_hi = std::max(n_hi, row[ix]);
                    if (ix > 0)
                        dn = std::max(dn, fabs(row[ix] - row[ix - 1]));
                    if (iy > 0)
                        dn = std::max(dn, fabs(row[ix] - row[ix - g.Nx]));
                }
            }
            if (!(n_lo - dn >= 0.25 && n_hi + dn <= 4.0 && dn / w_min <= 1e12 && w_min >= 1e-12))
                all_bounded = false;
            const double fy = g.y[0] >= 0.0 ? std::max(1.2, 1.0 + 2.0 * g.y[0] / (g.y[1] - g.y[0])) : 1.2;
            if (!(8.0 * 0.1 * (1.2 + fy) * dn <= 0.05 - 1e-5))
                ntest_proven = false;
            p->tab[(size_t) i].Nx    = g.Nx;
            p->tab[(size_t) i].Ny    = g.Ny;
            p->tab[(size_t) i].w_min = w_min;
            p->tab[(size_t) i].fy    = fy;
            p->tab[(size_t) i].off_node = (size_t) h.off_node;
        }
    }
    p->dz_bounded = beam->dz >= 1e-12 && beam->dz <= 1e6;
    if (!p->dz_bounded)
        all_bounded = false;
    p->tables_bounded = all_bounded;
    p->ntest_proven   = all_bounded && ntest_proven;
    p->march_prune    = (int) env_unsigned("RT_HIP_MARCH_PRUNE", 1, 0, 2);
    p->step_one_launch = env_unsigned("RT_HIP_STEP_ONE_LAUNCH", 0, 0, 1) == 1;
    if (tiny_spacing) {
        delete p;
        return fail_arg("rt_hip_plan_create: gain grid not strictly increasing, or spacing below 1e-30");
    }
    if (bad_index) {
        delete p;
        return fail_arg("rt_hip_plan_create: non-finite index of refraction");
    }
    const size_t off_blob = ab.put(blob.data(), blob.size());
    lap("pack");

#define PLAN_TRY(expr)                                   \
    do {                                                 \
        hipError_t e_ = (expr);                          \
        if (e_ != hipSuccess) {                          \
            rt_hip_plan_destroy(p);                      \
            return fail_hip(e_, #expr, __FILE__, __LINE__);        \
        }                                                \
    } while (0)

    if (ab.overflow) {
        delete p;
        return fail_arg("rt_hip_plan_create: internal error, the arena outgrew its computed capacity");
    }
    p->arena_bytes = align_up(ab.used, 256);
    PLAN_TRY(pool_alloc(device, (void **) &p->arena, p->arena_bytes));
    unsigned char *A = p->arena;
    p->gv_dev.assign((size_t) N, nullptr);
    for (int i = 1; i < N; i++) {
        dg[(size_t) i].gv    = reinterpret_cast<const float *>(A + off_gv[(size_t) i]);
        p->gv_dev[(size_t) i] = dg[(size_t) i].gv;
    }
    p->dv2_dev = reinterpret_cast<const double *>(A + off_bdv2);
    memcpy(ab.base + off_gain, dg.data(), sizeof(rt::DevGain) * (size_t) N);
    if (upload_q && ab.pinned) {
        const size_t bytes = ab.used;
        p->staging         = ab.release();
        p->upload_q        = upload_q;
        PLAN_TRY(hipMemcpyAsync(p->arena, p->staging, bytes, hipMemcpyHostToDevice, upload_q));
    } else {
        PLAN_TRY(hipMemcpy(p->arena, ab.base, ab.used, hipMemcpyHostToDevice));
    }
    lap("alloc + upload");

    rt::DevParams &P = p->P;
    P.N        = N;
    P.L        = L;
    P.K        = K;
    P.Kp       = Kp;
    P.method   = method;
    P.use_emis = use_emis ? 1 : 0;
    P.has_seed = seed ? 1 : 0;
    P.dz0      = (float) beam->dz;
    P.scale    = scale;
    P.beam.x   = reinterpret_cast<const double *>(A + off_bx);
    P.beam.y   = reinterpret_cast<const double *>(A + off_by);
    P.beam.a   = reinterpret_cast<const double *>(A + off_ba);
    P.beam.b   = reinterpret_cast<const double *>(A + off_bb);
    P.beam.dv  = reinterpret_cast<const double *>(A + off_bdv);
    P.beam.nx  = beam->nx;
    P.beam.ny  = beam->ny;
    P.beam.na  = beam->na;
    P.beam.nb  = beam->nb;
    P.beam.nv  = beam->nv;
    P.beam.dx  = beam->dx;
    P.beam.dy  = beam->dy;
    P.beam.da  = beam->da;
    P.beam.db  = beam->db;
    P.beam.inv_dx = 1.0 / beam->dx;
    P.beam.inv_dy = 1.0 / beam->dy;
    P.beam.inv_da = 1.0 / beam->da;
    P.beam.inv_db = 1.0 / beam->db;
    P.beam.g_first[0] = beam->x[0];
    P.beam.g_first[1] = beam->y[0];
    P.beam.g_first[2] = beam->a[0];
    P.beam.g_first[3] = beam->b[0];
    P.beam.g_last[0]  = beam->x[beam->nx - 1];
    P.beam.g_last[1]  = beam->y[beam->ny - 1];
    P.beam.g_last[2]  = beam->a[beam->na - 1];
    P.beam.g_last[3]  = beam->b[beam->nb - 1];
    if (seed) {
        for (int i = 0; i < 5; i++) {
            P.seed.x[i]   = reinterpret_cast<const double *>(A + off_sx[i]);
            P.seed.f[i]   = reinterpret_cast<const double *>(A + off_sf[i]);
            P.seed.dim[i] = seed->dim[i];
        }
        P.seed.f0 = seed->f0;
    }
    P.gain = reinterpret_cast<const rt::DevGain *>(A + off_gain);
    P.blob       = A + off_blob;
    P.blob_bytes = (unsigned) blob.size();
    if (const char *dbg = getenv("RT_HIP_DEBUG"))
        P.debug = (unsigned) strtoul(dbg, nullptr, 0);
    if (const char *ex = getenv("RT_HIP_EXACT_EMISSION"))
        P.exact_emis = atoi(ex) ? 1 : 0;

    p->beam_x.assign(beam->x, beam->x + beam->nx);
    p->beam_y.assign(beam->y, beam->y + beam->ny);
    p->beam_a.assign(beam->a, beam->a + beam->na);
    p->beam_b.assign(beam->b, beam->b + beam->nb);
    p->n_image = (size_t) beam->nx * (size_t) beam->ny * (size_t) beam->nv;
    p->n_iang  = (size_t) beam->na * (size_t) beam->nb;
    PLAN_TRY(pool_alloc(device, (void **) &p->ctl, sizeof(rt::DevCtl)));
    PLAN_TRY(hipEventCreate(&p->ev0));
    PLAN_TRY(hipEventCreate(&p->ev1));
    PLAN_TRY(hipEventCreate(&p->evm));
    P.rec_stride = (unsigned) align_up((size_t) L * RT_N_SUB * 12 + sizeof(rt::RecMeta), 16);
    P.c_cap      = 0.5f * 1.00001f;
    P.c_h1       = 0.5f * 0.1f;
    P.c_h3       = 0.5f * 0.05f;
    {
        float wmax = 0.0f;
        if (use_emis) {
            uint32_t umax          = 0;
            static const bool avx2 = __builtin_cpu_supports("avx2");
            for (int i = 1; i < N; i++) {
                const size_t n = (size_t) gain[i].Nx * (size_t) gain[i].Ny * (size_t) K;
                uint32_t m = 0, mall = 0;
                (avx2 ? magnitude_scan_avx2 : magnitude_scan_plain)(reinterpret_cast<const uint32_t *>(gain[i].gv), n, m, mall);
                umax = m > umax ? m : umax;
                if (mall >= 0x7f800000u)
                    p->gv_has_nan = true;
            }
            memcpy(&wmax, &umax, sizeof(wmax));
        }
        P.gs_cap = wmax > 0.0f ? 708.0f / wmax : FLT_MAX;
        if (!(P.gs_cap <= FLT_MAX))
            P.gs_cap = FLT_MAX;
    }
    P.ctl = p->ctl;
    *out  = p;
    lap("rest");
    return RT_OK;
}

int rtr::plan_build_seedset_tabs(rt_hip_plan *p)
{
    (void) hipFree(p->seedset_tab);
    p->seedset_tab = nullptr;
    for (int s = 0; s < RT_N_SEED_MAX; s++) {
        p->seedset_sf[s]  = nullptr;
        p->seedset_sin[s] = nullptr;
    }
    const rt::DevRays &R = p->P.rays;
    const int n_set = p->n_seed > 0 ? p->n_seed : p->n_scan_seed > 0 ? p->n_scan_seed : p->n_spec_seed;
    const bool ase_grid = p->P.use_emis && n_set > 0 && !R.list && R.gx && p->P.method != 1;
    if (n_set < 1 || (!R.sf && !ase_grid))
        return RT_OK;
    const size_t nn = (size_t) R.ngx + (size_t) R.ngy + (size_t) R.nga + (size_t) R.ngb;
    const size_t per_seed = align_up(nn * sizeof(double) + nn, 256);
    HIP_TRY(dev_malloc((void **) &p->seedset_tab, per_seed * (size_t) n_set));
    for (int s = 0; s < n_set; s++) {
        double *sf           = reinterpret_cast<double *>(p->seedset_tab + per_seed * (size_t) s);
        unsigned char *flags = reinterpret_cast<unsigned char *>(sf + nn);
        const int rc         = launch_seed_tab(p->seed_set[s], R, nn, sf, flags);
        if (rc != RT_OK)
            return rc;
        p->seedset_sf[s]  = sf;
        p->seedset_sin[s] = flags;
    }
    HIP_TRY(hipDeviceSynchronize());
    return RT_OK;
}

void rtr::plan_stage_outputs(rt_hip_plan *p)
{
    constexpr size_t ctl_tail = offsetof(rt::DevCtl, failure_code), ctl_bytes = sizeof(rt::DevCtl) - ctl_tail;
    if (!p || !p->ran || !p->last_stream)
        return;
    if (p->last_step && (p->last_step_lent || p->last_records.n_rec() > 0))
        return;
    const double *big    = p->last_step ? p->step_dev : p->last_image;
    const size_t n_big   = p->last_step ? p->step_doubles : p->n_image;
    const size_t off_ang = align_up(ctl_bytes, 256), off_img = off_ang + align_up(p->n_iang * sizeof(double), 256);
    const size_t total   = off_img + n_big * sizeof(double);
    if (total > ((size_t) 4 << 20))
        return;
    if (p->out_staging && p->out_staging_bytes < total) {
        pinned_free(p->out_staging);
        p->out_staging = nullptr;
    }
    if (!p->out_staging) {
        void *h = nullptr;
        if (pinned_alloc(&h, total) != hipSuccess)
            return;
        p->out_staging       = static_cast<unsigned char *>(h);
        p->out_staging_bytes = total;
    }
    hipError_t e = hipMemcpyAsync(p->out_staging, reinterpret_cast<const unsigned char *>(p->ctl) + ctl_tail, ctl_bytes,
                                  hipMemcpyDeviceToHost, p->last_stream);
    if (e == hipSuccess)
        e = hipMemcpyAsync(p->out_staging + off_ang, p->last_iang, p->n_iang * sizeof(double), hipMemcpyDeviceToHost, p->last_stream);
    if (e == hipSuccess)
        e = hipMemcpyAsync(p->out_staging + off_img, big, n_big * sizeof(double), hipMemcpyDeviceToHost, p->last_stream);
    if (e != hipSuccess) {
        (void) hipGetLastError();
        return;
    }
    p->out_staged = true;
}

int rtr::plan_set_rays_deferred(rt_hip_plan *p, const rt_ray *rays, size_t n_rays)
{
    if (n_rays > MAX_LIST_RAYS)
        return fail_arg("ray list of 2^32 - 4096 rays or more: split the call");
    HIP_TRY(hipSetDevice(p->device));
    plan_quiesce(p);
    pool_free(p->device, p->rays_dev);
    pool_free(p->device, p->tan_dev);
    p->rays_dev = nullptr;
    p->tan_dev  = nullptr;
    if (n_rays) {
        HIP_TRY(pool_alloc(p->device, (void **) &p->rays_dev, n_rays * sizeof(rt_ray)));
        HIP_TRY(pool_alloc(p->device, (void **) &p->tan_dev, n_rays * 2 * sizeof(float)));
    }
    p->P.exclusive  = 0;
    p->P.own_cells  = 0;
    p->P.rays       = {};
    p->P.rays.list  = p->rays_dev;
    p->P.rays.sxy   = p->tan_dev;
    p->P.rays.count = n_rays;
    p->n_rays       = n_rays;
    p->host_rays    = n_rays ? rays : nullptr;
    return RT_OK;
}

extern "C" {

int rt_hip_plan_set_rays(rt_hip_plan *p, const rt_ray *rays, size_t n_rays)
{
    if (!p || (n_rays && !rays))
        return fail_arg("rt_hip_plan_set_rays: NULL argument");
    if (n_rays > MAX_LIST_RAYS)
        return fail_arg("rt_hip_plan_set_rays: 2^32 - 4096 rays or more: split the call");
    HIP_TRY(hipSetDevice(p->device));
    plan_quiesce(p);
    pool_free(p->device, p->rays_dev);
    p->rays_dev = nullptr;
    if (n_rays) {
        HIP_TRY(pool_alloc(p->device, (void **) &p->rays_dev, n_rays * sizeof(rt_ray)));
        HIP_TRY(hipMemcpy(p->rays_dev, rays, n_rays * sizeof(rt_ray), hipMemcpyHostToDevice));
    }
    pool_free(p->device, p->tan_dev);
    p->tan_dev = nullptr;
    if (n_rays) {
        HIP_TRY(pool_alloc(p->device, (void **) &p->tan_dev, n_rays * 2 * sizeof(float)));
        if (tan_mode(p->device) == 2) {
            std::vector<float> h(n_rays * 2);
            host_tangents(rays, n_rays, h.data());
            HIP_TRY(hipMemcpy(p->tan_dev, h.data(), h.size() * sizeof(float), hipMemcpyHostToDevice));
        } else {
            const int rc = launch_tan(p->rays_dev, (unsigned long long) n_rays, p->tan_dev, nullptr);
            if (rc != RT_OK)
                return rc;
            HIP_TRY(hipDeviceSynchronize());
        }
    }
    p->P.exclusive  = 0;
    p->P.own_cells  = 0;
    p->P.rays       = {};
    p->P.rays.list  = p->rays_dev;
    p->P.rays.sxy   = p->tan_dev;
    p->P.rays.count = n_rays;
    p->n_rays       = n_rays;
    p->host_rays    = nullptr;
    return RT_OK;
}

int rt_hip_plan_set_ray_grid(rt_hip_plan *p, const double *gx, int ngx, const double *gy, int ngy,
                             const double *ga, int nga, const double *gb, int ngb, int64_t first,
                             int64_t stride, int64_t count)
{
    if (!p || !gx || !gy || !ga || !gb || ngx < 1 || ngy < 1 || nga < 1 || ngb < 1)
        return fail_arg("rt_hip_plan_set_ray_grid: bad grid");
    const int64_t total = (int64_t) ngx * ngy * nga * ngb;
    if (total > 0x7fffffffLL)
        return fail_arg("rt_hip_plan_set_ray_grid: more than 2^31 rays");
    if (first < 0 || stride < 1 || count < 0 || (count > 0 && first + (count - 1) * stride >= total))
        return fail_arg("rt_hip_plan_set_ray_grid: ray range outside the grid");
    HIP_TRY(hipSetDevice(p->device));
    plan_quiesce(p);
    pool_free(p->device, p->grid_dev);
    p->grid_dev     = nullptr;
    (void) hipFree(p->seedtab_dev);
    p->seedtab_dev  = nullptr;
    const size_t nn = (size_t) ngx + (size_t) ngy + (size_t) nga + (size_t) ngb;
    const size_t nt = (size_t) nga + (size_t) ngb;
    std::vector<double> h(nn + (nt + 1) / 2);
    memcpy(h.data(), gx, sizeof(double) * (size_t) ngx);
    memcpy(h.data() + ngx, gy, sizeof(double) * (size_t) ngy);
    memcpy(h.data() + ngx + ngy, ga, sizeof(double) * (size_t) nga);
    memcpy(h.data() + ngx + ngy + nga, gb, sizeof(double) * (size_t) ngb);
    {
        std::vector<float> ht(nt);
        for (int k = 0; k < nga; k++)
            ht[(size_t) k] = tanf(1e-3f * (float) ga[k]);
        for (int m = 0; m < ngb; m++)
            ht[(size_t) nga + (size_t) m] = tanf(1e-3f * (float) gb[m]);
        memcpy(h.data() + nn, ht.data(), nt * sizeof(float));
    }
    HIP_TRY(pool_alloc(p->device, (void **) &p->grid_dev, h.size() * sizeof(double)));
    HIP_TRY(hipMemcpy(p->grid_dev, h.data(), h.size() * sizeof(double), hipMemcpyHostToDevice));
    pool_free(p->device, p->tan_dev);
    p->tan_dev            = nullptr;
    const float *tan_grid = reinterpret_cast<const float *>(p->grid_dev + nn);
    p->host_rays   = nullptr;
    rt::DevRays &R = p->P.rays;
    R              = {};
    R.list         = nullptr;
    R.tan_a        = tan_grid;
    R.tan_b        = tan_grid + nga;
    R.gx           = p->grid_dev;
    R.gy           = p->grid_dev + ngx;
    R.ga           = p->grid_dev + ngx + ngy;
    R.gb           = p->grid_dev + ngx + ngy + nga;
    R.ngx          = ngx;
    R.ngy          = ngy;
    R.nga          = nga;
    R.ngb          = ngb;
    R.first        = first;
    R.stride       = stride;
    R.count        = (unsigned long long) count;
    p->n_rays      = (unsigned long long) count;
    {
        const int divisors[3] = { ngb, nga, ngy };
        for (int t = 0; t < 3; t++)
            magic_u31((unsigned) divisors[t], R.div_mul[t], R.div_sh[t]);
    }
    if (p->P.has_seed && p->P.method != 1) {
        HIP_TRY(dev_malloc((void **) &p->seedtab_dev, nn * sizeof(double) + nn));
        unsigned char *flags = reinterpret_cast<unsigned char *>(p->seedtab_dev + nn);
        const int rc = launch_seed_tab(p->P.seed, R, nn, p->seedtab_dev, flags);
        if (rc != RT_OK)
            return rc;
        HIP_TRY(hipDeviceSynchronize());
        R.sf  = p->seedtab_dev;
        R.sin = flags;
    }
    auto same = [](const std::vector<double> &v, const double *g, int n) {
        if ((int) v.size() != n)
            return false;
        for (int i = 0; i < n; i++) {
            const float a = (float) v[(size_t) i], b = (float) g[i];
            if (memcmp(&a, &b, sizeof(float)) != 0)
                return false;
        }
        return true;
    };
    auto own_cell = [](const std::vector<double> &g, double d) { return grid_points_in_own_cells(g.data(), (int) g.size(), d); };
    p->P.own_cells = (p->P.method == 1 && same(p->beam_x, gx, ngx) && same(p->beam_y, gy, ngy) && same(p->beam_a, ga, nga) &&
                      same(p->beam_b, gb, ngb) && own_cell(p->beam_x, p->P.beam.dx) && own_cell(p->beam_y, p->P.beam.dy) &&
                      own_cell(p->beam_a, p->P.beam.da) && own_cell(p->beam_b, p->P.beam.db) &&
                      !getenv("RT_HIP_NO_OWN_CELLS"))
                         ? 1u
                         : 0u;
    p->P.exclusive = (p->P.own_cells && p->P.use_emis && nga == 1 && ngb == 1 && first == 0 && stride == 1 && count == total) ? 1u : 0u;
    return plan_build_seedset_tabs(p);
}

int rt_hip_plan_set_exact_emission(rt_hip_plan *p, int on)
{
    if (!p)
        return fail_arg("rt_hip_plan_set_exact_emission: NULL plan");
    p->P.exact_emis = on ? 1 : 0;
    return RT_OK;
}

int rt_hip_plan_set_step_factor(rt_hip_plan *p, double c)
{
    if (!p || !(c > 0.0) || !(c < 1.0))
        return fail_arg("rt_hip_plan_set_step_factor: c must be in (0, 1)");
    const float cf = (float) c;
    p->P.c_cap     = cf * 1.00001f;
    p->P.c_h1      = cf * 0.1f;
    p->P.c_h3      = cf * 0.05f;
    return RT_OK;
}

int rt_hip_plan_set_debug(rt_hip_plan *p, unsigned bits)
{
    if (!p)
        return fail_arg("rt_hip_plan_set_debug: NULL plan");
    p->P.debug = bits;
    return RT_OK;
}
// ... 1044 lines not shown
int rt_hip_plan_set_spectra_seeds(rt_hip_plan *p, int n_seed, const rt_seed *seeds) { return seeds_set(p, SET_SPECTRA_SEEDS, n_seed, seeds, nullptr); }
int rt_hip_plan_set_spectra_ase_seeds(rt_hip_plan *p, int n_seed, const rt_seed *seeds)
{
    return seeds_set(p, SET_SPECTRA_ASE_SEEDS, n_seed, seeds, nullptr);
}

int rt_hip_plan_set_length_spectra_ase_seeds(rt_hip_plan *p, int n_seed, const rt_seed *seeds)
{
    return seeds_set(p, SET_LSPEC_ASE_SEEDS, n_seed, seeds, nullptr);
}

int rt_hip_plan_kernel_ms(rt_hip_plan *p, float *ms)
{
    if (!p || !p->ran || !ms)
        return fail_arg("rt_hip_plan_kernel_ms: plan has not run");
    HIP_TRY(hipSetDevice(p->device));
    HIP_TRY(hipEventSynchronize(p->ev1));
    HIP_TRY(hipEventElapsedTime(ms, p->ev0, p->ev1));
    return RT_OK;
}

int rt_hip_plan_set_timing_ring(rt_hip_plan *p, int n_runs)
{
    if (!p || n_runs < 1 || n_runs > 4096)
        return fail_arg("rt_hip_plan_set_timing_ring: 1 .. 4096 runs");
    HIP_TRY(hipSetDevice(p->device));
    plan_quiesce(p);
    if (p->ring.empty()) {
        p->ring = { p->ev0, p->evm, p->ev1 };
    }
    while (p->ring.size() < (size_t) n_runs * 3) {
        hipEvent_t e = nullptr;
        HIP_TRY(hipEventCreate(&e));
        p->ring.push_back(e);
    }
    while (p->ring.size() > (size_t) n_runs * 3) {
        (void) hipEventDestroy(p->ring.back());
        p->ring.pop_back();
    }
    p->ev0  = p->ring[0];
    p->evm  = p->ring[1];
    p->ev1  = p->ring[2];
    p->runs = 0;
    p->ran  = false;
    return RT_OK;
}

int rt_hip_plan_ring_times(rt_hip_plan *p, float *march_ms, float *freq_ms, int max_runs, int *n_runs)
{
    if (!p || !march_ms || !freq_ms || !n_runs || max_runs < 0)
        return fail_arg("rt_hip_plan_ring_times: bad argument");
    *n_runs = 0;
    if (!p->ran || p->ring.empty())
        return RT_OK;
    HIP_TRY(hipSetDevice(p->device));
    HIP_TRY(hipStreamSynchronize(p->last_stream));
    const unsigned long long slots = p->ring.size() / 3;
    const unsigned long long have  = p->runs < slots ? p->runs : slots;
    const unsigned long long take  = have < (unsigned long long) max_runs ? have : (unsigned long long) max_runs;
    for (unsigned long long i = 0; i < take; i++) {
        const size_t slot = (size_t) ((p->runs - take + i) % slots) * 3;
        HIP_TRY(hipEventElapsedTime(&march_ms[i], p->ring[slot], p->ring[slot + 1]));
        HIP_TRY(hipEventElapsedTime(&freq_ms[i], p->ring[slot + 1], p->ring[slot + 2]));
    }
    *n_runs = (int) take;
    return RT_OK;
}

int rt_hip_plan_kernel_times(rt_hip_plan *p, float *march_ms, float *freq_ms)
{
    if (!p || !p->ran || !march_ms || !freq_ms)
        return fail_arg("rt_hip_plan_kernel_times: plan has not run");
    HIP_TRY(hipSetDevice(p->device));
    HIP_TRY(hipEventSynchronize(p->ev1));
    HIP_TRY(hipEventElapsedTime(march_ms, p->ev0, p->evm));
    HIP_TRY(hipEventElapsedTime(freq_ms, p->evm, p->ev1));
    if (p->last_fused && p->last_step)
        *freq_ms = 0.0f;
    return RT_OK;
}

int rt_hip_plan_last_fused(rt_hip_plan *p) { return p && p->ran && p->last_fused ? 1 : 0; }
int rt_hip_plan_last_march_instance(rt_hip_plan *p) { return p && p->ran ? p->last_march_inst : 0; }

double *rt_hip_plan_image_ptr(rt_hip_plan *p) { return p ? p->image_own : nullptr; }
double *rt_hip_plan_iang_ptr(rt_hip_plan *p) { return p ? p->iang_own : nullptr; }

int rt_hip_plan_fetch_probe(rt_hip_plan *p, float *gvl, float *evl, int32_t *ivl, rt_ray *ray2,
                            uint32_t *flags, uint32_t *steps)
{
    if (!p || !p->ran || !p->probe_on || !p->probe)
        return fail_arg("rt_hip_plan_fetch_probe: probe was not enabled for the last run");
    HIP_TRY(hipSetDevice(p->device));
    HIP_TRY(hipStreamSynchronize(p->last_stream));
    const size_t n = (size_t) p->n_rays, S = (size_t) p->P.L * RT_N_SUB;
    {
        std::vector<unsigned char> h(rt::rec_bytes(n, p->P.rec_stride));
        if (n)
            HIP_TRY(hipMemcpy(h.data(), p->rec, h.size(), hipMemcpyDeviceToHost));
        for (size_t r = 0; r < n; r++) {
            const unsigned char *rec = h.data();
            const rt::RecMeta *mt = reinterpret_cast<const rt::RecMeta *>(rec + rt::rec_meta_off((unsigned) r, (int) S, p->P.rec_stride));
            for (size_t q = 0; q < S; q++) {
                const rt::RecSlot sl = rt::rec_slot(rec, (unsigned) r, p->P.rec_stride, (int) q, (int) S, mt->flags_steps, p->P.method == 1);
                if (gvl)
                    gvl[r * S + q] = sl.g;
                if (evl)
                    evl[r * S + q] = sl.e;
                if (ivl)
                    ivl[r * S + q] = sl.c;
            }
        }
    }
    if (ray2)
        HIP_TRY(hipMemcpy(ray2, p->P.probe.ray2, n * sizeof(rt_ray), hipMemcpyDeviceToHost));
    if (flags)
        HIP_TRY(hipMemcpy(flags, p->P.probe.flags, n * 4, hipMemcpyDeviceToHost));
    if (steps)
        HIP_TRY(hipMemcpy(steps, p->P.probe.steps, n * 4, hipMemcpyDeviceToHost));
    return RT_OK;
}

}

struct LoopRecords {
    ScanNeed scan        = SCANS_OFF;
    int n_seed           = 0;
    const rt_seed *seeds = nullptr;
    bool ase             = false;
    const double *scales = nullptr;
    bool rows() const { return scan != SCANS_OFF || ase; }
};
static int loop_records(rt_hip_plan *p, const LoopRecords &o)
{
    int rc = rt_hip_plan_enable_step(p, 1);
    if (rc == RT_OK && o.scan != SCANS_OFF)
        rc = scan_switch(p, o.scan == SUFFIX_SCAN_ON ? "rt_hip_plan_enable_suffix_scan" : "rt_hip_plan_enable_length_scan", o.scan == SUFFIX_SCAN_ON, 1);
    if (rc == RT_OK && o.n_seed > 0)
        rc = seeds_set(p, !o.ase ? (o.scan == SUFFIX_SCAN_ON ? SET_SUFFIX_SEEDS : SET_SCAN_SEEDS) : o.scan == SUFFIX_SCAN_ON ? SET_SUFFIX_ASE_SEEDS : o.scan == LENGTH_SCAN_ON ? SET_SCAN_ASE_SEEDS : SET_ASE_SEEDS,
                       o.n_seed, o.seeds, o.scales);
    return rc;
}
static int loop_check(const char *who, bool beam_ok, bool out_ok, const rt_ray *rays, size_t n_rays, bool seeds_ok = true)
{
    auto fail = [&](const char *what) { return fail_arg((std::string(who) + what).c_str()); };
    if (!beam_ok)
        return fail(": NULL beam");
    if (!out_ok)
        return fail(": NULL output");
    if (!rays && n_rays)
        return fail(": NULL ray list");
    if (n_rays > MAX_LIST_RAYS)
        return fail(": 2^32 - 4096 rays or more: split the call");
    if (!seeds_ok)
        return fail(": n_seed must be 1 .. RT_N_SEED_MAX, with seeds");
    return RT_OK;
}

static int host_pointer_loop(int device, int N, const rt_beam *beam, const rt_gain *gain, const rt_seed *seed,
                             int method, const rt_ray *rays, size_t n_rays, double scale, double *image, double *E_v, double *nf,
                             double *I_ang, unsigned int *failure_code, rt_ray *failed_rays, int max_failed,
                             int *n_failed, rt_stats *stats, const LoopRecords &o = LoopRecords())
{
    const bool step = image == nullptr;
    static const bool timing = getenv("RT_HIP_TIMING") != nullptr;
    auto t_prev = std::chrono::steady_clock::now();
// ... 258 lines not shown
```

### raytrace-miniapp_amd/csrc/rt_run_shape.h

```cpp
#pragma once

#include "rt_records.h"

#include <cstdlib>
#include <cstring>
#include <functional>

namespace rtr {

struct RunFacts {
    int cu_count              = 0;
    size_t lds_limit          = 0;
    unsigned long long n_rays = 0;
    unsigned n_tiles          = 0;
    size_t blob_bytes         = 0;
    int K = 0, Kp = 0, L = 0;
    size_t n_iang             = 0;
    int rays_per_pixel        = 0;
    int n_seed                = 0;
    float c_h3                = 0.0f;
    int march_prune           = 1;
    int method                = 0;
    unsigned safe = 0, debug = 0;
    bool use_emis = false, own_cells = false, exclusive = false, path_on = false, spectra_on = false, step_on = false,
         step_one_launch = false, probe_on = false, has_ray_list = false, host_rays = false, tables_bounded = false,
         ntest_proven = false, gv_has_nan = false;
    bool scan_on = false;
    bool length_spectra_on = false;
    bool scan_march() const { return scan_on || length_spectra_on; }
    bool rscan() const { return scan_march() && method == 1; }
    bool s6() const { return L * RT_N_SUB == 6; }
};

constexpr unsigned KNOB_UNSET = ~0u;
inline unsigned knob(unsigned k, unsigned def, unsigned hi = ~0u) { return k == KNOB_UNSET ? def : (k > hi ? hi : k); }

struct Tuning {
    bool march_global;
    bool march_ieee;
    unsigned upload_slices;
    unsigned fused;
    unsigned fused_seed;
    unsigned march_threads;
    unsigned march_mode;
    unsigned march_chunk;
    unsigned march_park;
    unsigned march_spin_limit;
    unsigned late_x10, late2_x10, late_waves, late_cap;
    unsigned fused_rows;
    unsigned fused_nodes;
    unsigned fused_split;
    unsigned fused_consumers;
    unsigned fused_consumers_first;
    unsigned freq_wg_waves;
    unsigned freq_min_rows;
    unsigned freq_wgs;
    unsigned step_serial;
};

inline Tuning read_tuning()
{
    Tuning t;
    const char *force       = getenv("RT_HIP_MARCH");
    t.march_global          = force && strcmp(force, "global") == 0;
    t.march_ieee            = getenv("RT_HIP_MARCH_IEEE") != nullptr;
    t.upload_slices         = env_unsigned("RT_HIP_UPLOAD_SLICES", KNOB_UNSET, 1, 8);
    t.fused                 = env_unsigned("RT_HIP_FUSED", 1, 1, 2);
    t.fused_seed            = env_unsigned("RT_HIP_FUSED_SEED", 0, 0, 1);
    t.march_threads         = env_unsigned("RT_HIP_MARCH_THREADS", KNOB_UNSET, 64, 1024);
    t.march_mode            = env_unsigned("RT_HIP_MARCH_MODE", 3, 0, 4);
    t.march_chunk           = env_unsigned("RT_HIP_MARCH_CHUNK", KNOB_UNSET, 1, 4096);
    t.march_park            = env_unsigned("RT_HIP_MARCH_PARK", 12, 1, 64);
    t.march_spin_limit      = env_unsigned("RT_HIP_MARCH_SPIN_LIMIT", 1u << 24, 1024, 0x7fffffffu);
    t.late_x10              = env_unsigned("RT_HIP_LATE_X10", 32, 0, 1000);
    t.late2_x10             = env_unsigned("RT_HIP_LATE2_X10", 60, 0, 1000);
    t.late_waves            = env_unsigned("RT_HIP_LATE_WAVES", 4, 0, 16);
    t.late_cap              = env_unsigned("RT_HIP_LATE_CAP", 20, 0, 100);
    t.fused_rows            = env_unsigned("RT_HIP_FUSED_ROWS", 7, 4, 16);
    t.fused_nodes           = env_unsigned("RT_HIP_FUSED_NODES", KNOB_UNSET, 0, 4096);
    t.fused_split           = env_unsigned("RT_HIP_FUSED_SPLIT", 1, 1, 3);
    t.fused_consumers       = env_unsigned("RT_HIP_FUSED_CONSUMERS", KNOB_UNSET, 0, 4096);
    t.fused_consumers_first = env_unsigned("RT_HIP_FUSED_CONSUMERS_FIRST", 0, 0, 1);
    t.freq_wg_waves         = env_unsigned("RT_HIP_FREQ_WG_WAVES", (unsigned) rt::FREQ_WG_WAVES, 1, (unsigned) rt::FREQ_WG_WAVES);
    t.freq_min_rows         = env_unsigned("RT_HIP_FREQ_MIN_ROWS", 7, 0, 16);
    t.freq_wgs              = env_unsigned("RT_HIP_FREQ_WGS", KNOB_UNSET, 1, 16);
    t.step_serial           = env_unsigned("RT_HIP_STEP_SERIAL", 0, 0, 1);
    return t;
}

inline unsigned one_wg_per_cu(unsigned long long items, unsigned per_wg, int cu_count)
{
    const unsigned long long want = (items + per_wg - 1) / per_wg;
    return (unsigned) (want < (unsigned long long) cu_count ? want : (unsigned long long) cu_count);
}
inline unsigned fetch_shift_of(unsigned long long grid_waves)
{
    unsigned sh = 0;
    while ((1ull << sh) < 2ull * grid_waves)
        sh++;
    return sh;
}
inline unsigned march_chunk(unsigned long long rays, unsigned grid, unsigned bthr)
{
    unsigned long long ch = grid ? rays / ((unsigned long long) grid * (bthr / 64) * 8) : 64;
    ch                    = ch < 64 ? 64 : (ch > 192 ? 192 : ch);
    return (unsigned) ((ch + 15) / 16 * 16);
}

enum RunKind { RUN_TWO_KERNELS = 0, RUN_IMAGE_ONE_LAUNCH = 1, RUN_STEP_ONE_LAUNCH = 2 };

struct RunShape {
    bool lds_tab      = false;
    unsigned n_launch = 1;
    RunKind kind      = RUN_TWO_KERNELS;
    unsigned bthr = 0;
    int mode = 0, opt = 0, last_march_inst = 0;
    bool bounded = false;
    size_t mlds  = 0;
    unsigned grid = 0, chunk = 0, park = 0, spin_limit = 0, no_skip = 0;
    unsigned late_first = 0, late_waves = 0, late_chunks = 0;
    bool occupancy_asked = false;
    bool emis = false;
    int maxq = 0, nslot = 0;
    rt::FusedLay lay = {};
    size_t flds = 0, tile_links = 0;
    unsigned fgrid = 0, fetch_shift = 0;
};

using Occupancy = std::function<int(const RunShape &s)>;

inline void late_zone(RunShape &s, const Tuning &t, unsigned long long n_rays, unsigned grid, unsigned waves_per_wg, unsigned first_marching_wave,
                      unsigned x10)
{
    s.late_first  = first_marching_wave;
    s.late_waves  = t.late_waves < waves_per_wg ? t.late_waves : waves_per_wg;
    s.late_chunks = 0;
    if (x10 == 0 || s.late_waves == 0 || s.chunk == 0)
        return;
    unsigned long long rays      = (unsigned long long) grid * s.late_waves * 64ull * x10 / 10ull;
    const unsigned long long cap = n_rays * t.late_cap / 100ull;
    rays                         = rays > cap ? cap : rays;
    s.late_chunks                = (unsigned) (rays / s.chunk);
}

inline bool one_launch_fits(RunShape &s, const RunFacts &f, const Tuning &t, bool step)
{
    const unsigned nw = s.bthr / 64;
    const bool emis   = s.emis;
    s.maxq  = emis && f.rays_per_pixel >= 64 ? 2 : 3;
    s.nslot = emis ? 0 : (int) t.fused_rows;
    size_t per_wave = (size_t) rt::fused_wave_doubles(s.maxq) + (size_t) s.nslot * (size_t) rt::freq_row_stride(f.Kp);
    if (step)
        per_wave = (size_t) 4 * rt::XP_ROW;
    rt::FusedLay &lay = s.lay;
    lay.off_exp  = (unsigned) align_up(f.blob_bytes, 16);
    lay.off_iang = lay.off_exp + 2u * rt::EXP_TAB * (unsigned) sizeof(double);
    lay.off_ctl  = lay.off_iang + (unsigned) (((f.n_iang + 1) & ~(size_t) 1) * sizeof(double));
    if (step)
        lay.off_ctl = lay.off_iang + rt::fused_step_ev_off((int) f.n_iang) + (unsigned) ((size_t) f.Kp * sizeof(double));
    lay.off_rem   = lay.off_ctl + 16u;
    lay.off_nodes = lay.off_rem + nw * 32u * (unsigned) sizeof(unsigned);
    {
        const unsigned long long wgs = one_wg_per_cu(f.n_rays, s.bthr, f.cu_count);
        unsigned long long cap       = wgs ? 2ull * ((unsigned long long) f.n_tiles / wgs + 1) + 32 : 64;
        cap                          = cap < 64 ? 64 : (cap > 1024 ? 1024 : cap);
        if (!emis)
            cap = cap > 256 ? 256 : cap;
        lay.node_cap = knob(t.fused_nodes, (unsigned) cap);
    }
    lay.off_buf = (unsigned) align_up(lay.off_nodes + lay.node_cap * 2u * (unsigned) sizeof(unsigned), 16);
    size_t room = f.lds_limit > lay.off_buf ? (f.lds_limit - lay.off_buf) / (per_wave * sizeof(double)) : 0;
    if (!emis && room < 5 && s.nslot > 5) {
        s.nslot  = 5;
        per_wave = (size_t) rt::fused_wave_doubles(s.maxq) + (size_t) s.nslot * (size_t) rt::freq_row_stride(f.Kp);
        room     = f.lds_limit > lay.off_buf ? (f.lds_limit - lay.off_buf) / (per_wave * sizeof(double)) : 0;
    }
    lay.per_wave = (unsigned) per_wave;
    lay.n_free   = (unsigned) (room < nw ? room : nw);
    s.flds       = (size_t) lay.off_buf + (size_t) lay.n_free * per_wave * sizeof(double);
    return (emis ? 2 * lay.n_free >= nw : (lay.n_free >= 3 && nw >= 8)) && (size_t) (nw - lay.n_free) * per_wave * sizeof(double) <= f.blob_bytes;
}

inline RunShape run_shape(const RunFacts &f, const Tuning &t, const Occupancy &occupancy)
{
    RunShape s;
    s.lds_tab = f.blob_bytes + 8 * 1024 <= f.lds_limit && !t.march_global;
    s.n_launch = (f.host_rays && f.n_rays >= (2ull << 20)) ? 3u : 1u;
    if (f.host_rays)
        s.n_launch = knob(t.upload_slices, s.n_launch);
    const bool iang_fits  = f.n_iang * sizeof(double) <= 32 * 1024;
    const bool fused_emis = f.use_emis && f.method == 1 && f.own_cells && f.rays_per_pixel >= 32;
    const bool fused_gain = !f.use_emis && !f.has_ray_list && t.fused_seed == 1;
    const bool fused_cand = s.lds_tab && s.n_launch == 1 && f.n_rays > 0 && !f.path_on && !f.spectra_on && !f.length_spectra_on && !f.step_on && !f.probe_on && f.debug == 0 &&
                            (fused_emis || fused_gain) && !f.exclusive && f.safe == 0 && iang_fits && t.fused == 1;
    const bool step_cand = f.step_on && f.step_one_launch && s.lds_tab && s.n_launch == 1 && f.n_rays > 0 && f.use_emis && f.method == 1 &&
                           f.own_cells && !f.probe_on && !f.path_on && !f.spectra_on && f.debug == 0 && f.safe == 0 && !f.exclusive &&
                           f.n_seed == 0 && !f.scan_on && iang_fits && t.fused == 1;
    s.bthr = s.lds_tab ? 1024u : 256u;
    if (s.lds_tab && !fused_cand && !step_cand) {
        const unsigned long long per_cu_rays = f.cu_count ? f.n_rays / (unsigned long long) f.cu_count : 0;
        s.bthr = per_cu_rays >= 4ull * 1024 ? 1024u : (per_cu_rays >= 2560ull ? 768u : 512u);
    }
    s.bthr = knob(t.march_threads, s.bthr, s.lds_tab ? 1024 : 256) / 64 * 64;
    s.mlds = s.lds_tab ? f.blob_bytes : 0;
    s.bounded = f.tables_bounded && f.c_h3 >= 1e-8f && !t.march_ieee;
    s.mode = (f.use_emis && f.method == 1 && !f.path_on) ? 1 : 0;
    if (!f.use_emis && f.method == 2 && !f.path_on)
        s.mode = (int) t.march_mode;
    const unsigned long long launch_rays = f.n_rays / s.n_launch;
    const bool prune_h24 = f.march_prune == 2 || (f.cu_count && launch_rays / (unsigned long long) f.cu_count >= 8192ull);
    s.opt = (s.bounded && f.march_prune && f.ntest_proven) ? (rt::MARCH_OPT_PRUNE | rt::MARCH_OPT_NO_NTEST | (prune_h24 ? rt::MARCH_OPT_PRUNE_H24 : 0)) : 0;
    if (f.scan_march()) {
        s.mode = f.rscan() ? (f.use_emis ? 1 : 0) : 3;
        s.opt  = rt::MARCH_OPT_SCAN;
    }
    s.last_march_inst = (s.bounded ? 1 : 0) | (s.opt << 1);
    int per_cu = 1;
    if (!s.lds_tab || (2 * s.mlds + 1024 <= f.lds_limit && s.bthr <= 512)) {
        s.occupancy_asked = true;
        per_cu            = occupancy(s);
    }
    if (per_cu < 1)
        per_cu = 1;
    const unsigned long long want = ((unsigned long long) f.n_rays + s.bthr - 1) / s.bthr;
    const unsigned long long cap  = (unsigned long long) f.cu_count * (unsigned) per_cu;
    s.grid       = (unsigned) (want < cap ? want : cap);
    s.chunk      = knob(t.march_chunk, march_chunk(f.n_rays, s.grid, s.bthr));
    s.park       = t.march_park;
    s.spin_limit = t.march_spin_limit;
    s.no_skip    = f.gv_has_nan ? 1u : 0u;
    s.emis       = f.use_emis;
    if ((fused_cand || step_cand) && s.grid > 0 && one_launch_fits(s, f, t, step_cand)) {
        const unsigned nw = s.bthr / 64;
        rt::FusedLay &lay = s.lay;
        s.kind       = step_cand ? RUN_STEP_ONE_LAUNCH : RUN_IMAGE_ONE_LAUNCH;
        s.tile_links = 4 * (size_t) f.n_tiles;
        lay.split  = t.fused_split == 2 ? 0u : (t.fused_split == 3 ? 2u : 1u);
        lay.k_part = f.K >= 32 && s.emis ? (unsigned) (((f.K + 3) / 4 + 3) / 4 * 4) : 0u;
        lay.n_consumers = knob(t.fused_consumers, s.emis ? nw / 4 : (lay.n_free < nw / 4 ? lay.n_free : nw / 4), nw > 1 ? nw - 1 : 0);
        if (lay.n_consumers >= nw)
            lay.n_consumers = nw - 1;
        lay.consumers_first = t.fused_consumers_first;
        s.chunk = (s.chunk + 32) / 64 * 64;
        s.chunk = s.chunk < 64 ? 64 : s.chunk;
        s.fgrid = one_wg_per_cu(f.n_rays, s.bthr, f.cu_count);
        if (s.emis)
            late_zone(s, t, f.n_rays, s.fgrid, nw - lay.n_consumers, lay.consumers_first ? lay.n_consumers : 0u, t.late_x10);
        s.fetch_shift = fetch_shift_of((unsigned long long) s.grid * nw);
        return s;
    }
    if (s.n_launch == 1 && s.lds_tab && s.grid > 0)
        late_zone(s, t, f.n_rays, s.grid, s.bthr / 64, 0u, t.late2_x10);
    return s;
}

inline RecordSet record_set(const RunFacts &f)
{
    RecordSet r;
    if (!f.step_on || f.path_on || f.spectra_on)
        return r;
    r.kind   = f.rscan() ? (f.n_seed > 0 ? (f.use_emis ? REC_RSCAN_ASE_SEEDS : REC_RSCAN_SEEDS) : REC_RSCAN) : f.scan_on ? (f.n_seed > 0 ? (f.use_emis ? REC_SCAN_ASE_SEEDS : REC_SCAN_SEEDS) : REC_SCAN) : f.n_seed > 0 ? (f.use_emis ? REC_ASE_SEEDS : REC_SEEDS) : REC_NONE;
    r.n_seed = f.n_seed;
    r.L      = f.scan_on ? f.L : 0;
    return r;
}

inline RowSet row_set(const RunFacts &f)
{
    RowSet r;
    if (f.path_on || (!f.spectra_on && !f.length_spectra_on))
        return r;
    r.kind   = f.spectra_on ? (f.n_seed > 0 ? (f.use_emis ? ROWS_SPEC_ASE_SEEDS : ROWS_SPEC_SEEDS) : ROWS_SPEC)
                            : f.n_seed > 0 ? (f.use_emis ? ROWS_LSPEC_ASE_SEEDS : ROWS_LSPEC_SEEDS) : ROWS_LSPEC;
    r.n_seed = f.n_seed;
    r.L      = r.lengths() ? f.L : 0;
    r.n_rays = (size_t) f.n_rays;
    return r;
}

inline PassKind pass_kind(const RunFacts &f)
{
    if (f.path_on)
        return PASS_PATH;
    if (row_set(f).any())
        return row_set(f).pass_kind();
    return f.step_on ? record_set(f).pass_kind() : PASS_FREQ;
}

struct PassShape {
    int wg_waves = 0, nslot = 0;
    bool in_lds  = false;
    size_t lds   = 0;
    unsigned grid = 0, fetch_shift = 0;
};

inline void freq_pass_shape(PassShape &s, const RunFacts &f, const Tuning &t)
{
    const bool emis = f.use_emis, excl = f.use_emis && f.exclusive;
    const int waves = emis ? rt::FREQ_WAVES : rt::FREQ_WAVES_SEED;
    s.wg_waves      = (int) t.freq_wg_waves;
    int wg_per_cu   = waves * 4 / s.wg_waves;
    wg_per_cu       = wg_per_cu < 1 ? 1 : wg_per_cu;
    auto lds_of     = [&](int rows) { return rt::freq_lds_doubles(s.in_lds, (int) f.n_iang, excl, rows, f.Kp, s.wg_waves) * sizeof(double); };
    auto rows_that_fit = [&](size_t budget) {
        int rows = 0;
        while (rows < 16 && lds_of(rows + 1) + 1024 <= budget)
            rows++;
        return rows;
    };
    if (!excl) {
        s.nslot = rows_that_fit(f.lds_limit / (size_t) wg_per_cu);
        if (!emis && s.nslot < (int) t.freq_min_rows && wg_per_cu > 1) {
            wg_per_cu--;
            s.nslot = rows_that_fit(f.lds_limit / (size_t) wg_per_cu);
        }
// ... 46 lines not shown
```

### raytrace-miniapp_amd/csrc/rt_runtime.h

```cpp
#pragma once

#include "rt_device.h"
#include "rt_records.h"
#include "rt_spec.h"
#include "rt_step.h"

#include <chrono>
#include <cstddef>
#include <string>
#include <vector>

namespace rtr {

struct History {
    int n_steps = 0;
    bool bound  = false;
    RecordSet recs;
    int n_rec = 0;
    int nv = 0, nx = 0, ny = 0, na = 0, nb = 0;
    unsigned char *dev = nullptr;
    rt_hip_history_layout lay = {};
    std::vector<unsigned char> filled;
    hipEvent_t ev      = nullptr;
    bool pending       = false;
    hipStream_t stream = nullptr;
};

}

struct rt_hip_plan {
    int device         = 0;
    int cu_count       = 0;
    rt::DevParams P    = {};
    unsigned char *arena = nullptr;
    size_t arena_bytes = 0;
    void *staging        = nullptr;
    hipStream_t upload_q = nullptr;
    unsigned char *out_staging = nullptr;
    bool out_staged            = false;
    size_t out_staging_bytes   = 0;
    rt_ray *rays_dev   = nullptr;
    double *grid_dev   = nullptr;
    float *tan_dev     = nullptr;
    double *seedtab_dev = nullptr;
    std::vector<double> beam_x, beam_y, beam_a, beam_b;
    unsigned char *rec = nullptr;
    bool path_on       = false;
    float *path_dev    = nullptr;
    int32_t *path_err  = nullptr;
    size_t path_rays   = 0;
    bool spectra_on    = false;
    rtr::RowSet last_rows;
    unsigned spec_sel  = 0;
    unsigned spec_last = 0;
    rt::SpecOut spec[2] = {};
    size_t spec_rays[2] = { 0, 0 };
    bool lspec_on      = false;
    bool lspec_first_done = false;
    rt::SpecOut lspec  = {};
    unsigned char *lspec_dev = nullptr;
    size_t lspec_bytes = 0;
    int n_spec_seed    = 0;
    bool step_on       = false;
    bool last_step     = false;
    double *step_dev   = nullptr;
    size_t step_doubles = 0;
    rt::StepOut step   = {};
    double *step_ev_lent = nullptr, *step_nf_lent = nullptr;
    bool last_step_lent  = false;
    int n_seed      = 0;
    int n_scan_seed = 0;
    rt::DevSeed seed_set[RT_N_SEED_MAX] = {};
    unsigned char *seedset_arena = nullptr;
    unsigned char *seedset_tab   = nullptr;
    const double *seedset_sf[RT_N_SEED_MAX]         = {};
    const unsigned char *seedset_sin[RT_N_SEED_MAX] = {};
    double ase_scale[RT_N_SEED_MAX] = {};
    bool scan_on          = false;
    unsigned char *scan_bnd = nullptr;
    size_t scan_bnd_bytes = 0;
    double *recs_dev    = nullptr;
    size_t recs_doubles = 0;
    size_t recs_stride = 0, recs_nf_off = 0, recs_ang_off = 0;
    rtr::RecordSet last_records;
    size_t bad_word = 1;
    size_t rec_bytes   = 0;
    hipEvent_t evm     = nullptr;
    const rt_ray *host_rays = nullptr;
    double *image_own  = nullptr;
    double *iang_own   = nullptr;
    rt::DevCtl *ctl    = nullptr;
    size_t n_image = 0, n_iang = 0;
    unsigned long long n_rays = 0;
    bool probe_on        = false;
    unsigned char *probe = nullptr;
    size_t probe_rays    = 0;
    hipEvent_t ev0 = nullptr, ev1 = nullptr;
    hipStream_t last_stream = nullptr;
    hipStream_t queued_stream = nullptr;
    bool queued = false;
    double *last_image = nullptr, *last_iang = nullptr;
    bool ran = false;
    std::vector<hipEvent_t> ring;
    unsigned long long runs = 0;
    bool repeated = false;
    unsigned char *bad_dev = nullptr;
    size_t bad_rays        = 0;
    std::chrono::steady_clock::time_point t_created;
    std::vector<const float *> gv_dev;
    const double *dv2_dev = nullptr;
    bool gv_has_nan       = false;
    bool tables_bounded   = false;
    bool ntest_proven     = false;
    int march_prune       = 1;
    int last_march_inst   = 0;
    unsigned *tile_next   = nullptr;
    size_t tile_next_n    = 0;
    bool last_fused       = false;
    bool step_one_launch  = false;
    size_t lds_limit      = 0;
    struct TableShape {
        int Nx = 0, Ny = 0;
        double w_min = 0.0;
        double fy    = 1.2;
        size_t off_node = 0;
    };
// ... 95 lines not shown
```

Measured before the change: 31.22 billion.

## Stage grid ray start tables in LDS alongside gain blob

Packs the grid ray start coordinates and angle tangents as float tables placed after the gain blob and copies them into LDS. Rays can then read their start point from shared memory instead of reading double global arrays. The run-shape logic reserves the extra LDS only when it does not change occupancy, free wave slots or node capacity, trimming the node cap when needed. This adds LDS pressure and more planning complexity, and the float conversion of gx/gy, which the old path also did, is now done on the host.

```diff
diff --git a/include/rt_hip.h b/include/rt_hip.h
--- a/include/rt_hip.h
+++ b/include/rt_hip.h
@@ -144,6 +144,11 @@
 } rt_hip_run_shape;
 int rt_hip_debug_run_shape(const rt_hip_run_facts *facts, rt_hip_run_shape *out);
 
+int rt_hip_plan_last_start_lds(rt_hip_plan *plan);
+int rt_hip_debug_run_shape_start(const rt_hip_run_facts *facts, unsigned long long start_points, rt_hip_run_shape *out, unsigned *start_off);
+int rt_hip_debug_pack_start_tables(const double *gx, int ngx, const double *gy, int ngy, const float *tan_a, int nga, const float *tan_b,
+                                   int ngb, float *out, unsigned long long *bytes);
+
 int rt_hip_plan_set_timing_ring(rt_hip_plan *plan, int n_runs);
 int rt_hip_plan_ring_times(rt_hip_plan *plan, float *march_ms, float *freq_ms, int max_runs, int *n_runs);
 
diff --git a/raytrace-miniapp_amd/backend.py b/raytrace-miniapp_amd/backend.py
--- a/raytrace-miniapp_amd/backend.py
+++ b/raytrace-miniapp_amd/backend.py
@@ -685,6 +685,9 @@
 
     def last_march_instance(self) -> int:
         return int(self.hl.lib.rt_hip_plan_last_march_instance(self._h))
+
+    def last_start_lds(self) -> int:
+        return int(self.hl.lib.rt_hip_plan_last_start_lds(self._h))
 
     def set_timing_ring(self, n_runs: int) -> "Plan":
         self.hl.check(self.hl.lib.rt_hip_plan_set_timing_ring(self._h, int(n_runs)), "rt_hip_plan_set_timing_ring")
diff --git a/raytrace-miniapp_amd/cabi.py b/raytrace-miniapp_amd/cabi.py
--- a/raytrace-miniapp_amd/cabi.py
+++ b/raytrace-miniapp_amd/cabi.py
@@ -358,6 +358,14 @@
     if hasattr(lib, "rt_hip_debug_run_shape"):
         lib.rt_hip_debug_run_shape.argtypes = [P(RtRunFacts), P(RtRunShape)]
         lib.rt_hip_debug_run_shape.restype = C.c_int
+    if hasattr(lib, "rt_hip_plan_last_start_lds"):
+        lib.rt_hip_plan_last_start_lds.argtypes = [vp]
+        lib.rt_hip_plan_last_start_lds.restype = C.c_int
+        lib.rt_hip_debug_run_shape_start.argtypes = [P(RtRunFacts), C.c_ulonglong, P(RtRunShape), P(C.c_uint)]
+        lib.rt_hip_debug_run_shape_start.restype = C.c_int
+        lib.rt_hip_debug_pack_start_tables.argtypes = [c_double_p, C.c_int, c_double_p, C.c_int, P(C.c_float), C.c_int,
+                                                       P(C.c_float), C.c_int, P(C.c_float), P(C.c_ulonglong)]
+        lib.rt_hip_debug_pack_start_tables.restype = C.c_int
     if hasattr(lib, "rt_hip_plan_enable_length_scan"):
         lib.rt_hip_plan_enable_length_scan.argtypes = [vp, C.c_int]
         lib.rt_hip_plan_enable_length_scan.restype = C.c_int
@@ -494,6 +502,7 @@
     "rt_hip_plan_set_spectra_ase_seeds", "rt_hip_plan_fetch_full_spectra", "rt_hip_plan_full_spectra_ptrs",
     "rt_hip_plan_set_length_spectra_ase_seeds", "rt_hip_plan_fetch_full_length_spectra", "rt_hip_plan_full_length_spectra_ptrs",
     "rt_hip_plan_set_step_one_launch", "rt_hip_debug_run_shape",
+    "rt_hip_plan_last_start_lds", "rt_hip_debug_run_shape_start", "rt_hip_debug_pack_start_tables",
     "rt_hip_plan_history_create", "rt_hip_plan_history_append", "rt_hip_plan_history_ptrs", "rt_hip_plan_history_sum_ptrs",
     "rt_hip_plan_history_fetch", "rt_hip_plan_history_fetch_sum", "rt_hip_plan_history_info", "rt_hip_debug_history_layout",
     "rt_hip_plan_set_debug", "rt_hip_plan_destroy",
diff --git a/raytrace-miniapp_amd/csrc/rt_blob_pack.h b/raytrace-miniapp_amd/csrc/rt_blob_pack.h
--- a/raytrace-miniapp_amd/csrc/rt_blob_pack.h
+++ b/raytrace-miniapp_amd/csrc/rt_blob_pack.h
@@ -7,6 +7,24 @@
 #include "rt_device.h"
 
 namespace rt {
+
+inline size_t start_tab_pack(std::vector<float> &out, const double *gx, int ngx, const double *gy, int ngy, const float *tan_a, int nga,
+                             const float *tan_b, int ngb)
+{
+    const size_t nn = (size_t) ngx + (size_t) ngy + (size_t) nga + (size_t) ngb, padded = (nn + 3) / 4 * 4;
+    out.clear();
+    if (padded * sizeof(float) > START_TAB_MAX)
+        return 0;
+    out.assign(padded, 0.0f);
+    float *q = out.data();
+    for (int i = 0; i < ngx; i++)
+        *q++ = (float) gx[i];
+    for (int j = 0; j < ngy; j++)
+        *q++ = (float) gy[j];
+    memcpy(q, tan_a, sizeof(float) * (size_t) nga);
+    memcpy(q + nga, tan_b, sizeof(float) * (size_t) ngb);
+    return padded * sizeof(float);
+}
 
 inline BlobGain blob_pack_length(std::vector<unsigned char> &blob, size_t i, int Nx, int Ny, const double *x, const double *y,
                                  const double *n, const float *g0, const float *E0, bool &tiny_spacing, bool &bad_index)
diff --git a/raytrace-miniapp_amd/csrc/rt_device.h b/raytrace-miniapp_amd/csrc/rt_device.h
--- a/raytrace-miniapp_amd/csrc/rt_device.h
+++ b/raytrace-miniapp_amd/csrc/rt_device.h
@@ -37,6 +37,8 @@
     double hi;
     double rh;
 };
+
+constexpr unsigned START_TAB_MAX = 4096;
 
 struct DevSeed {
     const double *x[5];
diff --git a/raytrace-miniapp_amd/csrc/rt_launch.hip b/raytrace-miniapp_amd/csrc/rt_launch.hip
--- a/raytrace-miniapp_amd/csrc/rt_launch.hip
+++ b/raytrace-miniapp_amd/csrc/rt_launch.hip
@@ -209,6 +209,7 @@
     f.n_rays          = p->n_rays;
     f.n_tiles         = P.n_tiles;
     f.blob_bytes      = P.blob_bytes;
+    f.start_bytes     = P.rays.list ? 0 : p->start_bytes;
     f.K               = P.K;
     f.Kp              = P.Kp;
     f.L               = P.L;
@@ -667,6 +668,13 @@
         P.pad_march[0]             = (unsigned) (b & 0xffffffffull);
         P.pad_march[1]             = (unsigned) (b >> 32);
     }
+    P.pad_march[2] = P.pad_march[3] = 0;
+    const unsigned x4 = s.start_off / 4, y4 = x4 + (unsigned) P.rays.ngx, a4 = y4 + (unsigned) P.rays.ngy, b4 = a4 + (unsigned) P.rays.nga;
+    if (s.start_off && b4 < 0x10000u) {
+        P.pad_march[2] = x4 | (y4 << 16);
+        P.pad_march[3] = a4 | (b4 << 16);
+        P.blob_bytes   = (unsigned) s.mlds;
+    }
     return P;
 }
 
@@ -746,6 +754,7 @@
     if (rc != RT_OK)
         return rc;
     p->last_march_inst = s.last_march_inst;
+    p->last_start_off  = s.start_off;
     if ((rc = ensure_buffers(p, s, stream)) != RT_OK)
         return rc;
     HIP_TRY(hipEventRecord(p->ev0, stream));
@@ -767,7 +776,7 @@
 
 extern "C" {
 
-int rt_hip_debug_run_shape(const rt_hip_run_facts *facts, rt_hip_run_shape *out)
+static int debug_run_shape(const rt_hip_run_facts *facts, unsigned long long start_points, rt_hip_run_shape *out, unsigned *start_off)
 {
     if (!facts || !out || facts->size != sizeof(rt_hip_run_facts) || out->size != sizeof(rt_hip_run_shape))
         return fail_arg("rt_hip_debug_run_shape: NULL argument or a size field that is not this library's sizeof");
@@ -779,6 +788,10 @@
     f.n_rays          = facts->n_rays;
     f.n_tiles         = facts->n_tiles;
     f.blob_bytes      = (size_t) facts->blob_bytes;
+    {
+        const unsigned long long bytes = (start_points + 3) / 4 * 16;
+        f.start_bytes = (facts->has_ray_list || bytes > rt::START_TAB_MAX) ? 0 : (size_t) bytes;
+    }
     f.K               = facts->K;
     f.Kp              = facts->Kp;
     f.L               = facts->L;
@@ -820,6 +833,8 @@
     out->opt             = s.opt;
     out->last_march_inst = s.last_march_inst;
     out->mlds            = s.mlds;
+    if (start_off)
+        *start_off = s.start_off;
     out->grid            = s.grid;
     out->chunk           = s.chunk;
     out->park            = s.park;
@@ -872,6 +887,15 @@
     return RT_OK;
 }
 
+int rt_hip_debug_run_shape(const rt_hip_run_facts *facts, rt_hip_run_shape *out) { return debug_run_shape(facts, 0, out, nullptr); }
+int rt_hip_debug_run_shape_start(const rt_hip_run_facts *facts, unsigned long long start_points, rt_hip_run_shape *out, unsigned *start_off)
+{
+    if (!start_off)
+        return fail_arg("rt_hip_debug_run_shape_start: NULL argument");
+    *start_off = 0;
+    return debug_run_shape(facts, start_points, out, start_off);
+}
+
 #ifdef RT_WAVETIMES
 int rt_hip_debug_wavetimes(unsigned long long *summary8, unsigned long long *end8192, unsigned long long *dry8192)
 {
diff --git a/raytrace-miniapp_amd/csrc/rt_march.hip b/raytrace-miniapp_amd/csrc/rt_march.hip
--- a/raytrace-miniapp_amd/csrc/rt_march.hip
+++ b/raytrace-miniapp_amd/csrc/rt_march.hip
@@ -47,6 +47,34 @@
             ta = R.tan_a[k];
             tb = R.tan_b[m];
         }
+    }
+}
+
+template <bool LDS_TAB>
+__device__ __forceinline__ void load_start(const DevRays &R, const unsigned char *lds_raw, unsigned where_xy, unsigned where_tan,
+                                           unsigned ridx, float &x, float &y, float &ta, float &tb)
+{
+    if (R.list) {
+        const rt_ray ray = R.list[ridx];
+        x                = ray.x;
+        y                = ray.y;
+        ta               = R.sxy[2 * (size_t) ridx];
+        tb               = R.sxy[2 * (size_t) ridx + 1];
+        return;
+    }
+    unsigned i, j, k, m;
+    grid_index(R, ridx, i, j, k, m);
+    if (LDS_TAB && where_xy != 0u) {
+        const float *t = reinterpret_cast<const float *>(lds_raw);
+        x              = t[(where_xy & 0xffffu) + i];
+        y              = t[(where_xy >> 16) + j];
+        ta             = t[(where_tan & 0xffffu) + k];
+        tb             = t[(where_tan >> 16) + m];
+    } else {
+        x  = (float) R.gx[i];
+        y  = (float) R.gy[j];
+        ta = R.tan_a[k];
+        tb = R.tan_b[m];
     }
 }
 
@@ -832,11 +860,8 @@
                 if (!BOUNDED && __ballot(got) != 0ull)
                     spin = 0;
                 if (got) {
-                    rt_ray ray;
                     float ta = 0, tb = 0;
-                    load_ray(P.rays, ridx, ray, ta, tb, true);
-                    px = ray.x;
-                    py = ray.y;
+                    load_start<LDS_TAB>(P.rays, lds_raw, P.pad_march[2], P.pad_march[3], ridx, px, py, ta, tb);
                     pz = 0.0f;
                     sx = ta;
                     sy = tb;
diff --git a/raytrace-miniapp_amd/csrc/rt_plan.hip b/raytrace-miniapp_amd/csrc/rt_plan.hip
--- a/raytrace-miniapp_amd/csrc/rt_plan.hip
+++ b/raytrace-miniapp_amd/csrc/rt_plan.hip
@@ -285,7 +285,7 @@
             capacity += piece(cells * kp * sizeof(float));
             blob_bytes += sizeof(rt::Interval) * ((size_t) gain[i].Nx + (size_t) gain[i].Ny) + sizeof(rt::Node) * cells;
         }
-        capacity += piece(blob_bytes);
+        capacity += piece(blob_bytes + rt::START_TAB_MAX);
         capacity += piece(sizeof(double) * (size_t) beam->nx) + piece(sizeof(double) * (size_t) beam->ny) +
                     piece(sizeof(double) * (size_t) beam->na) + piece(sizeof(double) * (size_t) beam->nb) + 2 * piece(sizeof(double) * kp);
         if (seed)
@@ -394,6 +394,8 @@
         delete p;
         return fail_arg("rt_hip_plan_create: non-finite index of refraction");
     }
+    const size_t blob_bytes = blob.size();
+    blob.resize(blob_bytes + rt::START_TAB_MAX, 0);
     const size_t off_blob = ab.put(blob.data(), blob.size());
     lap("pack");
 
@@ -476,7 +478,7 @@
     }
     P.gain = reinterpret_cast<const rt::DevGain *>(A + off_gain);
     P.blob       = A + off_blob;
-    P.blob_bytes = (unsigned) blob.size();
+    P.blob_bytes = (unsigned) blob_bytes;
     if (const char *dbg = getenv("RT_HIP_DEBUG"))
         P.debug = (unsigned) strtoul(dbg, nullptr, 0);
     if (const char *ex = getenv("RT_HIP_EXACT_EMISSION"))
@@ -604,6 +606,7 @@
     p->P.exclusive  = 0;
     p->P.own_cells  = 0;
     p->P.rays       = {};
+    p->start_bytes  = 0;
     p->P.rays.list  = p->rays_dev;
     p->P.rays.sxy   = p->tan_dev;
     p->P.rays.count = n_rays;
@@ -646,6 +649,7 @@
     p->P.exclusive  = 0;
     p->P.own_cells  = 0;
     p->P.rays       = {};
+    p->start_bytes  = 0;
     p->P.rays.list  = p->rays_dev;
     p->P.rays.sxy   = p->tan_dev;
     p->P.rays.count = n_rays;
@@ -678,6 +682,9 @@
     memcpy(h.data() + ngx, gy, sizeof(double) * (size_t) ngy);
     memcpy(h.data() + ngx + ngy, ga, sizeof(double) * (size_t) nga);
     memcpy(h.data() + ngx + ngy + nga, gb, sizeof(double) * (size_t) ngb);
+    std::vector<float> &start = p->start_host;
+    size_t start_bytes        = 0;
+    p->start_bytes            = 0;
     {
         std::vector<float> ht(nt);
         for (int k = 0; k < nga; k++)
@@ -685,9 +692,18 @@
         for (int m = 0; m < ngb; m++)
             ht[(size_t) nga + (size_t) m] = tanf(1e-3f * (float) gb[m]);
         memcpy(h.data() + nn, ht.data(), nt * sizeof(float));
+        start_bytes = rt::start_tab_pack(start, gx, ngx, gy, ngy, ht.data(), nga, ht.data() + nga, ngb);
     }
     HIP_TRY(pool_alloc(p->device, (void **) &p->grid_dev, h.size() * sizeof(double)));
     HIP_TRY(hipMemcpy(p->grid_dev, h.data(), h.size() * sizeof(double), hipMemcpyHostToDevice));
+    if (start_bytes) {
+        unsigned char *dst = const_cast<unsigned char *>(p->P.blob) + p->P.blob_bytes;
+        if (p->upload_q)
+            HIP_TRY(hipMemcpyAsync(dst, start.data(), start_bytes, hipMemcpyHostToDevice, p->upload_q));
+        else
+            HIP_TRY(hipMemcpy(dst, start.data(), start_bytes, hipMemcpyHostToDevice));
+        p->start_bytes = start_bytes;
+    }
     pool_free(p->device, p->tan_dev);
     p->tan_dev            = nullptr;
     const float *tan_grid = reinterpret_cast<const float *>(p->grid_dev + nn);
@@ -1898,6 +1914,18 @@
 
 int rt_hip_plan_last_fused(rt_hip_plan *p) { return p && p->ran && p->last_fused ? 1 : 0; }
 int rt_hip_plan_last_march_instance(rt_hip_plan *p) { return p && p->ran ? p->last_march_inst : 0; }
+int rt_hip_plan_last_start_lds(rt_hip_plan *p) { return p && p->ran ? (int) p->last_start_off : 0; }
+int rt_hip_debug_pack_start_tables(const double *gx, int ngx, const double *gy, int ngy, const float *tan_a, int nga, const float *tan_b,
+                                   int ngb, float *out, unsigned long long *bytes)
+{
+    if (!gx || !gy || !tan_a || !tan_b || !out || !bytes || ngx < 1 || ngy < 1 || nga < 1 || ngb < 1)
+        return fail_arg("rt_hip_debug_pack_start_tables: bad argument");
+    std::vector<float> t;
+    *bytes = rt::start_tab_pack(t, gx, ngx, gy, ngy, tan_a, nga, tan_b, ngb);
+    if (*bytes)
+        memcpy(out, t.data(), (size_t) *bytes);
+    return RT_OK;
+}
 
 double *rt_hip_plan_image_ptr(rt_hip_plan *p) { return p ? p->image_own : nullptr; }
 double *rt_hip_plan_iang_ptr(rt_hip_plan *p) { return p ? p->iang_own : nullptr; }
diff --git a/raytrace-miniapp_amd/csrc/rt_run_shape.h b/raytrace-miniapp_amd/csrc/rt_run_shape.h
--- a/raytrace-miniapp_amd/csrc/rt_run_shape.h
+++ b/raytrace-miniapp_amd/csrc/rt_run_shape.h
@@ -14,6 +14,7 @@
     unsigned long long n_rays = 0;
     unsigned n_tiles          = 0;
     size_t blob_bytes         = 0;
+    size_t start_bytes        = 0;
     int K = 0, Kp = 0, L = 0;
     size_t n_iang             = 0;
     int rays_per_pixel        = 0;
@@ -56,6 +57,7 @@
     unsigned freq_min_rows;
     unsigned freq_wgs;
     unsigned step_serial;
+    unsigned start_lds;
 };
 
 inline Tuning read_tuning()
@@ -85,6 +87,7 @@
     t.freq_min_rows         = env_unsigned("RT_HIP_FREQ_MIN_ROWS", 7, 0, 16);
     t.freq_wgs              = env_unsigned("RT_HIP_FREQ_WGS", KNOB_UNSET, 1, 16);
     t.step_serial           = env_unsigned("RT_HIP_STEP_SERIAL", 0, 0, 1);
+    t.start_lds             = env_unsigned("RT_HIP_START_LDS", 1, 0, 1);
     return t;
 }
 
@@ -117,6 +120,7 @@
     int mode = 0, opt = 0, last_march_inst = 0;
     bool bounded = false;
     size_t mlds  = 0;
+    unsigned start_off = 0;
     unsigned grid = 0, chunk = 0, park = 0, spin_limit = 0, no_skip = 0;
     unsigned late_first = 0, late_waves = 0, late_chunks = 0;
     bool occupancy_asked = false;
@@ -143,7 +147,7 @@
     s.late_chunks                = (unsigned) (rays / s.chunk);
 }
 
-inline bool one_launch_fits(RunShape &s, const RunFacts &f, const Tuning &t, bool step)
+inline bool one_launch_fits(RunShape &s, const RunFacts &f, const Tuning &t, bool step, size_t tab_bytes, size_t node_give = 0)
 {
     const unsigned nw = s.bthr / 64;
     const bool emis   = s.emis;
@@ -153,7 +157,7 @@
     if (step)
         per_wave = (size_t) 4 * rt::XP_ROW;
     rt::FusedLay &lay = s.lay;
-    lay.off_exp  = (unsigned) align_up(f.blob_bytes, 16);
+    lay.off_exp  = (unsigned) align_up(tab_bytes, 16);
     lay.off_iang = lay.off_exp + 2u * rt::EXP_TAB * (unsigned) sizeof(double);
     lay.off_ctl  = lay.off_iang + (unsigned) (((f.n_iang + 1) & ~(size_t) 1) * sizeof(double));
     if (step)
@@ -166,6 +170,9 @@
         cap                          = cap < 64 ? 64 : (cap > 1024 ? 1024 : cap);
         if (!emis)
             cap = cap > 256 ? 256 : cap;
+        const unsigned long long give = (node_give + 7) / 8;
+        if (t.fused_nodes == KNOB_UNSET && cap >= 64 + give)
+            cap -= give;
         lay.node_cap = knob(t.fused_nodes, (unsigned) cap);
     }
     lay.off_buf = (unsigned) align_up(lay.off_nodes + lay.node_cap * 2u * (unsigned) sizeof(unsigned), 16);
@@ -178,7 +185,19 @@
     lay.per_wave = (unsigned) per_wave;
     lay.n_free   = (unsigned) (room < nw ? room : nw);
     s.flds       = (size_t) lay.off_buf + (size_t) lay.n_free * per_wave * sizeof(double);
-    return (emis ? 2 * lay.n_free >= nw : (lay.n_free >= 3 && nw >= 8)) && (size_t) (nw - lay.n_free) * per_wave * sizeof(double) <= f.blob_bytes;
+    return (emis ? 2 * lay.n_free >= nw : (lay.n_free >= 3 && nw >= 8)) && (size_t) (nw - lay.n_free) * per_wave * sizeof(double) <= tab_bytes;
+}
+
+inline size_t start_tables_room(const RunFacts &f, const Tuning &t, bool lds_tab)
+{
+    if (!lds_tab || t.start_lds == 0 || f.start_bytes == 0 || f.start_bytes > rt::START_TAB_MAX)
+        return 0;
+    const size_t st = align_up(f.start_bytes, 16), both = f.blob_bytes + st;
+    if (both + 8 * 1024 > f.lds_limit || both / 4 >= 0x10000)
+        return 0;
+    if ((2 * f.blob_bytes + 1024 <= f.lds_limit) != (2 * both + 1024 <= f.lds_limit))
+        return 0;
+    return st;
 }
 
 inline RunShape run_shape(const RunFacts &f, const Tuning &t, const Occupancy &occupancy)
@@ -202,7 +221,9 @@
         s.bthr = per_cu_rays >= 4ull * 1024 ? 1024u : (per_cu_rays >= 2560ull ? 768u : 512u);
     }
     s.bthr = knob(t.march_threads, s.bthr, s.lds_tab ? 1024 : 256) / 64 * 64;
-    s.mlds = s.lds_tab ? f.blob_bytes : 0;
+    const size_t start = start_tables_room(f, t, s.lds_tab);
+    s.mlds      = s.lds_tab ? f.blob_bytes + start : 0;
+    s.start_off = start ? (unsigned) f.blob_bytes : 0u;
     s.bounded = f.tables_bounded && f.c_h3 >= 1e-8f && !t.march_ieee;
     s.mode = (f.use_emis && f.method == 1 && !f.path_on) ? 1 : 0;
     if (!f.use_emis && f.method == 2 && !f.path_on)
@@ -230,7 +251,16 @@
     s.spin_limit = t.march_spin_limit;
     s.no_skip    = f.gv_has_nan ? 1u : 0u;
     s.emis       = f.use_emis;
-    if ((fused_cand || step_cand) && s.grid > 0 && one_launch_fits(s, f, t, step_cand)) {
+    const RunShape two = s;
+    if ((fused_cand || step_cand) && s.grid > 0 && one_launch_fits(s, f, t, step_cand, f.blob_bytes)) {
+        s.start_off = 0;
+        RunShape with = two;
+        RunShape trimmed = two;
+        if (start && one_launch_fits(with, f, t, step_cand, f.blob_bytes + start) && with.lay.n_free == s.lay.n_free && with.nslot == s.nslot)
+            s = with;
+        else if (start && one_launch_fits(trimmed, f, t, step_cand, f.blob_bytes + start, start) && trimmed.lay.n_free == s.lay.n_free &&
+                 trimmed.nslot == s.nslot)
+            s = trimmed;
         const unsigned nw = s.bthr / 64;
         rt::FusedLay &lay = s.lay;
         s.kind       = step_cand ? RUN_STEP_ONE_LAUNCH : RUN_IMAGE_ONE_LAUNCH;
diff --git a/raytrace-miniapp_amd/csrc/rt_runtime.h b/raytrace-miniapp_amd/csrc/rt_runtime.h
--- a/raytrace-miniapp_amd/csrc/rt_runtime.h
+++ b/raytrace-miniapp_amd/csrc/rt_runtime.h
@@ -42,6 +42,9 @@
     rt_ray *rays_dev   = nullptr;
     double *grid_dev   = nullptr;
     float *tan_dev     = nullptr;
+    size_t start_bytes   = 0;
+    std::vector<float> start_host;
+    unsigned last_start_off = 0;
     double *seedtab_dev = nullptr;
     std::vector<double> beam_x, beam_y, beam_a, beam_b;
     unsigned char *rec = nullptr;
```

Result: no change. 31.38 billion, median of 6 (+0.5%).
